# pixray/pixray

Measured on AMD Instinct MI355X. Metric: optimisation iters/sec, VQGAN 256^2 + ViT-B/32 + 64 cutouts, higher is better.
Workload: dtype fp16

## Files before the change

include/prx.h:

```cpp
#ifndef PRX_H_
#define PRX_H_
#include <stddef.h>
#include <stdint.h>

#ifdef __cplusplus
extern "C" {
#endif

#define PRX_ABI_VERSION 3

typedef void* prx_stream_t;

const char* prx_last_error(void);
int prx_abi_version(void);
int prx_device_info(int* cu_count, char* arch_name, int arch_name_len);


#define PRX_ACT_NONE 0
#define PRX_ACT_QUICKGELU 1
#define PRX_ACT_MUL_DQUICKGELU 2
#define PRX_ACT_RELU 3
#define PRX_ACT_MUL_RELUMASK 4
#define PRX_ACT_RELUMASK_POST 5
#define PRX_ACT_GELU 6
#define PRX_ACT_MUL_DGELU 7
#define PRX_A_ROWMAJOR 0
#define PRX_A_CONV3X3 1

#define PRX_PREC_BF16 0
#define PRX_PREC_F32 1
#define PRX_PREC_F16 2

typedef struct prx_gemm_ctx prx_gemm_ctx;
prx_gemm_ctx* prx_gemm_ctx_create(void);
void prx_gemm_ctx_destroy(prx_gemm_ctx* c);

typedef struct prx_gemm_args {
    const void* A;
    int a_is_f32, a_mode, lda;
    const void* B;
    int ldb;
    int M, N, K;
    int H, W, Cin, up;
    float alpha;
    const float* bias_n;
    const float* bias_m;
    const void* aux;
    int ldaux;
    const float* resid;
    int ldr;
    int act;
    float* out_f32; int ldc_f32;
    void* out_bf16; void* out_bf16_pre; int ldc_bf16;
    int f32;
    int row16;
    prx_gemm_ctx* ctx;
} prx_gemm_args;
int prx_k_gemm(const prx_gemm_args* g, void* ws, size_t ws_bytes, prx_stream_t stream);
int prx_k_gemm_gn(const prx_gemm_args* g, double* gn_stats, int gn_gs, const float* gnb_x, const double* gnb_fstats,
                  const float* gnb_gamma, const float* gnb_beta, int gnb_swish, float gnb_eps, void* ws, size_t ws_bytes,
                  prx_stream_t stream);
long long prx_gemm_fit_spec_launches(void);
long long prx_gemm_row_launches(void);

int prx_k_groupnorm_fwd(const float* x, const float* gamma, const float* beta, double* stats, void* out_bf16,
                        float* out_f32, int NB, int P, int C, int swish, float eps, prx_stream_t s);
int prx_k_groupnorm_bwd(const float* g, const float* x, const float* gamma, const float* beta, const double* fstats,
                        double* bstats, const float* add, float* dx, int NB, int P, int C, int swish, float eps,
                        prx_stream_t s);
int prx_k_layernorm_fwd(const float* x, long long ldx, const float* gamma, const float* beta, void* out_bf16,
                        float* out_f32, float* mean, float* rstd, int rows, int C, float eps, prx_stream_t s);
int prx_k_layernorm_bwd(const float* g, long long ldg, const float* x, long long ldx, const float* gamma,
                        const float* mean, const float* rstd, const float* add, long long ldadd, float* dx,
                        long long lddx, int rows, int C, prx_stream_t s);
int prx_k_transpose_bf16(const void* in, int ldin, void* out, int ldout, int R, int C, prx_stream_t s);
int prx_k_softmax_rows(const float* S, int lds_, float scale, void* P, int ldp, void* PT, int ldpt, int rows, int cols,
                       prx_stream_t s);
int prx_k_softmax_rows_bwd(const void* P, int ldp, const float* dP, int lddp, float scale, void* dS, int ldds,
                           void* dST, int lddst, int rows, int cols, prx_stream_t s);
int prx_k_upsample2x_bwd(const float* hi, float* low, int NB, int Hl, int Wl, int C, prx_stream_t s);
int prx_k_nchw_to_nhwc(const float* in, float* out_f32, void* out_bf16, int NB, int C, int HW, int Cpad,
                       prx_stream_t s);
int prx_k_nhwc_to_nchw(const float* in, int ldc, float* out, int NB, int C, int HW, prx_stream_t s);
int prx_k_image_head_fwd(const float* x, int ldc, float* img, int NB, int C, int HW, prx_stream_t s);
int prx_k_image_head_bwd(const float* x, int ldc, const float* gimg, float* dx, void* dx_bf16, int ldo, int NB, int C,
                         int HW, prx_stream_t s);
int prx_k_mha_fwd(const void* qkv, void* out, int N, int T, int C, int heads, prx_stream_t s);
int prx_k_mha_bwd(const void* qkv, const void* dout, void* dqkv, int N, int T, int C, int heads, prx_stream_t s);

int prx_k_groupnorm_fwd_op(const void* x, const float* gamma, const float* beta, double* stats, void* out16, float* out_f32,
                           int NB, int P, int C, int swish, float eps, int zero_stats, int stats_ready, int h16, int s16,
                           prx_stream_t s);
int prx_k_groupnorm_bwd_op(const void* g, const void* x, const float* gamma, const float* beta, const double* fstats,
                           double* bstats, const void* add, float* dx, void* dx16, int NB, int P, int C, int swish, float eps,
                           int zero_stats, int stats_ready, int h16, int s16, prx_stream_t s);
int prx_k_layernorm_fwd_op(const void* x, long long ldx, const float* gamma, const float* beta, void* out16, float* out_f32,
                           float* mean, float* rstd, int rows, int C, float eps, int h16, int s16, prx_stream_t s);
int prx_k_layernorm_bwd_op(const void* g, long long ldg, const void* x, long long ldx, const float* gamma, const float* mean,
                           const float* rstd, const void* add, long long ldadd, float* dx, long long lddx, void* dx16,
                           long long lddxb, int rows, int C, int h16, int add_every, int s16, prx_stream_t s);
int prx_k_mha_fwd_op(const void* qkv, void* out, int N, int T, int C, int heads, int h16, prx_stream_t s);
int prx_k_mha_bwd_op(const void* qkv, const void* dout, void* dqkv, int N, int T, int C, int heads, int h16, prx_stream_t s);
int prx_k_mha_fwd_gen_op(const void* qkv, void* out, float* lse, int N, int T, int C, int heads, int h16, prx_stream_t s);
int prx_k_mha_bwd_gen_op(const void* qkv, const void* out, const void* dout, const float* lse, void* dqkv, int N, int T, int C,
                         int heads, int h16, prx_stream_t s);
int prx_k_mha_fwd_hd_op(const void* qkv, void* out, float* lse, int N, int T, int C, int heads, int h16, int head_cols, prx_stream_t s);
int prx_k_mha_bwd_hd_op(const void* qkv, const void* out, const void* dout, const float* lse, void* dqkv, int N, int T, int C,
                        int heads, int h16, int head_cols, prx_stream_t s);
int prx_k_mha_fwd_hdim_op(const void* qkv, void* out, float* lse, int N, int T, int C, int heads, int h16, int head_cols, int head_dim,
                          prx_stream_t s);
int prx_k_mha_bwd_hdim_op(const void* qkv, const void* out, const void* dout, const float* lse, void* dqkv, int N, int T, int C,
                          int heads, int h16, int head_cols, int head_dim, prx_stream_t s);
int prx_k_layernorm_fwd_rag_op(const void* x, long long ldx, const float* gamma, const float* beta, void* out16, float* out_f32,
                               float* mean, float* rstd, int rows, int C, float eps, int h16, int s16, prx_stream_t s);
int prx_k_layernorm_bwd_rag_op(const void* g, long long ldg, const void* x, long long ldx, const float* gamma, const float* mean,
                               const float* rstd, const void* add, long long ldadd, float* dx, long long lddx, void* dx16, long long lddxb,
                               int rows, int C, int h16, int add_every, int s16, prx_stream_t s);
int prx_k_vit_pad_heads(const float* qkv_w, float* qkv_w_pad, const float* out_w, float* out_w_pad, int width, int heads, int hd, int hp,
                        prx_stream_t s);
int prx_k_mha_fwd_causal_op(const void* qkv, void* out, int N, int T, int C, int heads, int h16, prx_stream_t s);
int prx_k_softmax_rows_op(const float* S, int lds_, float scale, void* P, int ldp, void* PT, int ldpt, int rows, int cols,
                          int prec, prx_stream_t s);
int prx_k_softmax_rows_bwd_op(const void* P, int ldp, const float* dP, int lddp, float scale, void* dS, int ldds, void* dST,
                              int lddst, int rows, int cols, int prec, prx_stream_t s);
int prx_k_transpose_op(const void* in, int ldin, void* out, int ldout, int R, int C, int f32, prx_stream_t s);
int prx_k_upsample2x_bwd_op(const void* hi, float* low, void* low16, int NB, int Hl, int Wl, int C, int h16, int s16,
                            prx_stream_t s);
int prx_k_nchw_to_nhwc_op(const float* in, float* out_f32, void* out16, int NB, int C, int HW, int Cpad, int h16, prx_stream_t s);
int prx_k_image_head_bwd_op(const float* x, int ldc, const float* gimg, float* dx, void* dx16, int ldo, int NB, int C, int HW,
                            int h16, const float* gscale, prx_stream_t s);
int prx_k_image_head_bwd_im2col(const float* x, int ldc, const float* gimg, void* col, int ldk, int C, int H, int W, int h16,
                                const float* gscale, prx_stream_t s);
int prx_k_grad_scale(const float* g, size_t n, float* part, int nparts, int target_log2, float* scale2, prx_stream_t s);
int prx_k_grad_scale_multi(const float* const* gs, const size_t* ns, int count, float* part, int nparts_each, int target_log2,
                           float* scale2, prx_stream_t s);
int prx_k_scale_dev(float* x, size_t n, const float* scale, void* out16, int h16, prx_stream_t s);
int prx_k_f32_to_op16(const float* in, void* out16, size_t n, int h16, prx_stream_t s);
int prx_k_add_f32(const float* a, const float* b, float* out, size_t n, prx_stream_t s);

int prx_k_rn_pack_conv3x3(const float* w, void* Wf, void* Wd, int Cout, int Cin, int prec, prx_stream_t s);
int prx_k_stem1_fwd(const float* cut, const float* mm, const float* w, const float* b, void* out, int N, int S, int CO, int prec,
                    prx_stream_t s);
int prx_k_stem1_bwd(const void* g, const float* w, float* dY, int N, int S, int CO, const float* oscale_dev, int prec, prx_stream_t s);
int prx_k_avgpool2_fwd(const void* x, void* out, int N, int H, int W, int C, int prec, prx_stream_t s);
int prx_k_avgpool2_bwd(const float* g, const void* mask, float* dx_f32, void* dx_op, int N, int H, int W, int C, int prec,
                       prx_stream_t s);
int prx_k_relu_mask(float* g, const void* out, void* g_op, size_t n, int prec, prx_stream_t s);
int prx_k_tokens_fwd(const float* x, const float* pos, void* t, int N, int P, int C, int prec, prx_stream_t s);
int prx_k_tokens_bwd(const float* dt, float* dx, int N, int P, int C, int prec, prx_stream_t s);
int prx_k_tok0_gather(const void* t, void* out, int N, int T, int C, int prec, prx_stream_t s);
int prx_k_tok0_scatter(const void* g0, void* dt, int N, int T, int C, int prec, prx_stream_t s);
int prx_k_cnx_pack_dw(const float* w, void* pack, int C, int prec, prx_stream_t s);
int prx_k_cnx_dwconv(const void* x, const void* pack, const float* bias, const float* add, void* out_op, float* out_f32, int N, int H,
                     int W, int C, int flip, int prec, prx_stream_t s);
int prx_k_cnx_space_to_depth(const void* in, void* out, int N, int H, int W, int C, int prec, prx_stream_t s);
int prx_k_cnx_depth_to_space(const void* in, void* out, int N, int H, int W, int C, int prec, prx_stream_t s);
int prx_k_cnx_avgpool_fwd(const void* x, float* out, int N, int HW, int C, int prec, prx_stream_t s);
int prx_k_cnx_avgpool_bwd(const float* g, float* dx_f32, void* dx_op, int N, int HW, int C, int prec, prx_stream_t s);
int prx_k_cnx_layernorm_fwd(const void* x, int x_f32, const float* gamma, const float* beta, void* out_op, float* out_f32, float* mean,
                            float* rstd, int rows, int C, float eps, int group, int prec, prx_stream_t s);
int prx_k_cnx_layernorm_bwd(const float* g, const void* x, int x_f32, const float* gamma, const float* mean, const float* rstd,
                            void* dx_op, float* dx_f32, int rows, int C, int group, int prec, prx_stream_t s);
int prx_k_minmax(const float* x, size_t n, float* part, int nparts, float* mm, prx_stream_t s);
int prx_k_patchify_fwd(const float* cut, const float* mm, void* A, int prec, int N, int S, int P, int T, float m0, float m1, float m2,
                       float s0, float s1, float s2, prx_stream_t s);
int prx_k_patchify_bwd_reduce(const float* cut, const float* mm, const float* dA, double* acc, int N, int S, int P, int T, float m0,
                              float m1, float m2, float s0, float s1, float s2, prx_stream_t s);
int prx_k_patchify_bwd_apply(const float* cut, const float* mm, const float* dA, const double* acc, float* gcut, int N, int S, int P,
                             int T, float m0, float m1, float m2, float s0, float s1, float s2, prx_stream_t s);
int prx_k_preproc_bwd_reduce(const float* cut, const float* mm, const float* dY, double* acc, int N, int S, prx_stream_t s);
int prx_k_preproc_bwd_apply(const float* cut, const float* mm, const float* dY, const double* acc, float* gcut, int N, int S,
                            prx_stream_t s);
int prx_k_pool_fwd(const float* img, float* pooled, int* argmax, const unsigned char* mask, int C, int H, int W, int S, prx_stream_t s);
int prx_k_pool_bwd(const float* g, const int* argmax, const unsigned char* mask, float* gimg, int C, int H, int W, int S, prx_stream_t s);
int prx_k_rescale_fwd(const float* pooled, float* base, int C, int S, int Hb, int Wb, prx_stream_t s);
int prx_k_rescale_bwd(const float* g_base, float* g_pooled, int C, int S, int Hb, int Wb, prx_stream_t s);
int prx_k_warp_a_fwd(const float* src, int Hs, int Ws, const double* desc, float* out, int n_cut, int Ha, int Wa, prx_stream_t s);
int prx_k_warp_a_bwd(const float* g, int Hs, int Ws, const double* desc, float* uv, float* gsrc_priv, float* gsrc, int n_cut, int Ha,
                     int Wa, int form, prx_stream_t s);
int prx_k_warp_b_fwd(const float* a, int Ha, int Wa, const double* desc, const float* noise, float* out, int n_cut, int S,
                     prx_stream_t s);
int prx_k_warp_b_bwd(const float* a, int Ha, int Wa, const double* desc, const float* g, float* grgb, float* uv, float* ga, int n_cut,
                     int S, float* maps_scratch, size_t maps_scratch_bytes, int form, prx_stream_t s);
int prx_cutout_bwd_separable(int on);
int prx_k_vgg_pack(const float* w, void* Wf, void* Wd, int Cout, int Cin, int CiP, int prec, prx_stream_t s);
int prx_k_vgg_input(const float* x, void* out, int HW, int prec, prx_stream_t s);
int prx_k_vgg_input_grad(const float* d, float* gx, int HW, const float* unscale, prx_stream_t s);
int prx_k_vgg_maxpool(const void* x, void* out, void* arg, int H, int W, int C, int prec, prx_stream_t s);
int prx_k_vgg_combine(const float* above, const void* arg, const float* gcap, const void* act, void* gpre, int H, int W, int C,
                      const float* gscale, int prec, prx_stream_t s);
int prx_k_pack_transpose_op(const float* in, void* out, int R, int C, int prec, prx_stream_t s);
int prx_k_vit_add_cls_pos(float* x, const float* cls, const float* pos, int N, int T, int W, prx_stream_t s);
int prx_k_vit_embed_tokens(const float* x, const float* cls, const float* pos, void* out, int out16, int N, int T, int W,
                           prx_stream_t s);
int prx_k_vit_gelu_f32(const float* t, float* io, size_t n, int bwd, prx_stream_t s);
int prx_k_vit_scale_f32(float* x, size_t n, float scale, int blocks, prx_stream_t s);
int prx_k_text_embed(const int* tokens, const float* emb, const float* pos, float* x, int* eot, int n, int ctx, int W, int vocab,
                     prx_stream_t s);
int prx_k_gather_rows(const float* x, const int* eot, float* out, int n, int ctx, int W, prx_stream_t s);
int prx_k_l2norm_fwd(const float* e, float* out, int n, int D, prx_stream_t s);
int prx_k_l2norm_bwd(const float* e, const float* g, float* de, int n, int D, prx_stream_t s);
int prx_k_vqgan_pack_conv3x3(const float* w, void* Wf, void* Wd, int Cout, int Cin, int CoP, int prec, prx_stream_t s);
int prx_k_vqgan_enc_pack_conv3x3(const float* w, void* Wf, int Cout, int Cin, int CiP, prx_stream_t s);
int prx_k_colminmax(const float* w, float* mn, float* mx, int rows, int D, prx_stream_t s);


typedef struct prx_vqgan prx_vqgan;
// ... 329 lines not shown
```

pixray_amd/csrc/api_core.hip:

```cpp
#include "common.h"
#include "gemm.h"
#include "../../include/prx.h"
#include <stdarg.h>
#include <stdio.h>
#include <string.h>
#include <stdlib.h>

static thread_local char g_err[1024] = "";

void prx_set_error(const char* fmt, ...) {
    va_list ap;
    va_start(ap, fmt);
    vsnprintf(g_err, sizeof(g_err), fmt, ap);
    va_end(ap);
}

int prx_xcd_local() {
    static const int v = getenv("PRX_XCD_LOCAL") ? atoi(getenv("PRX_XCD_LOCAL")) : 1;
    return v;
}

int prx_grad_target_log2() {
    static const int v = [] {
        const char* e = getenv("PRX_GRAD_TARGET_LOG2");
        int k = e ? atoi(e) : 4;
        return k < -8 ? -8 : (k > 14 ? 14 : k);
    }();
    return v;
}

extern "C" {

const char* prx_last_error(void) { return g_err; }

int prx_abi_version(void) { return PRX_ABI_VERSION; }

int prx_device_info(int* cu_count, char* arch_name, int arch_name_len) {
    int dev = 0;
    PRX_CHECK_HIP(hipGetDevice(&dev));
    hipDeviceProp_t p;
    PRX_CHECK_HIP(hipGetDeviceProperties(&p, dev));
    if (cu_count) *cu_count = p.multiProcessorCount;
    if (arch_name && arch_name_len > 0) {
        strncpy(arch_name, p.gcnArchName, arch_name_len - 1);
        arch_name[arch_name_len - 1] = 0;
    }
    return 0;
}

static int desc_of(const prx_gemm_args* g, GemmDesc& d) {
    PRX_REQUIRE(g != nullptr, "prx_k_gemm: null args");
    PRX_REQUIRE(prec_valid(g->f32), "prx_k_gemm: unknown operand precision %d", g->f32);
    d.f32 = prec_is_f32(g->f32); d.h16 = prec_is_h16(g->f32);
    d.A = g->A; d.a_is_f32 = g->a_is_f32; d.a_mode = g->a_mode; d.lda = g->lda;
    d.B = g->B; d.ldb = g->ldb;
    d.M = g->M; d.N = g->N; d.K = g->K;
    d.H = g->H; d.W = g->W; d.Cin = g->Cin; d.up = g->up;
    d.alpha = g->alpha;
    d.bias_n = g->bias_n; d.bias_m = g->bias_m;
    d.aux = g->aux; d.ldaux = g->ldaux;
    d.resid = g->resid; d.ldr = g->ldr;
    d.act = g->act;
    d.out_f32 = g->out_f32; d.ldc_f32 = g->ldc_f32;
    d.out_bf16 = g->out_bf16; d.out_bf16_pre = g->out_bf16_pre;
    d.ldc_bf16 = g->ldc_bf16;
    d.row16 = (short)(g->row16 & 3);
    return 0;
}
int prx_k_gemm(const prx_gemm_args* g, void* ws, size_t ws_bytes, prx_stream_t stream_) {
    GemmDesc d;
    int r = desc_of(g, d);
    if (r) return r;
    return prx_gemm_launch(d, (float*)ws, ws_bytes, (hipStream_t)stream_, (GemmCtx*)g->ctx);
}
int prx_k_gemm_gn(const prx_gemm_args* g, double* gn_stats, int gn_gs, const float* gnb_x, const double* gnb_fstats,
                  const float* gnb_gamma, const float* gnb_beta, int gnb_swish, float gnb_eps, void* ws, size_t ws_bytes,
                  prx_stream_t stream_) {
    GemmDesc d;
    int r = desc_of(g, d);
    if (r) return r;
    PRX_REQUIRE(gn_stats != nullptr, "prx_k_gemm_gn: null gn_stats");
    d.gn_stats = gn_stats; d.gn_gs = gn_gs;
    d.gnb_x = gnb_x; d.gnb_fstats = gnb_fstats; d.gnb_gamma = gnb_gamma; d.gnb_beta = gnb_beta; d.gnb_swish = gnb_swish; d.gnb_eps = gnb_eps;
    return prx_gemm_launch(d, (float*)ws, ws_bytes, (hipStream_t)stream_, (GemmCtx*)g->ctx);
}

prx_gemm_ctx* prx_gemm_ctx_create(void) { return (prx_gemm_ctx*)new GemmCtx(); }
void prx_gemm_ctx_destroy(prx_gemm_ctx* c) { delete (GemmCtx*)c; }
void prx_profile_gemm_enable(prx_gemm_ctx* c, int on) { prx_gemm_ctx_profile_enable((GemmCtx*)c, on); }
void prx_gemm_tile_override(prx_gemm_ctx* c, int bm, int bn, int splits) { prx_gemm_ctx_force_tile((GemmCtx*)c, bm, bn, splits); }
int prx_gemm_plan(prx_gemm_ctx* c, const prx_gemm_args* g, size_t ws_bytes, int n_cu, int* out) {
    GemmDesc d;
    int r = desc_of(g, d);
    if (r) return r;
    GemmPlan p;
    r = prx_gemm_plan_impl(d, (const GemmCtx*)c, n_cu, ws_bytes, true, &p);
    if (r) return r;
    const GemmLaunchPlan& l0 = p.launch[0], l1 = p.n_launch == 2 ? p.launch[1] : GemmLaunchPlan{};
    const int o[9] = {l0.family, l0.bm, l0.bn, l0.splits, p.rows_8p, p.n_launch == 2 ? (int)l1.family : -1, l1.bm, l1.bn, p.n_launch == 2 ? l1.splits : 0};
    memcpy(out, o, sizeof o);
    return 0;
}
int prx_gemm_plan_rows_8phase(prx_gemm_ctx* c, int M, int N, int K) {
    if (M <= 0 || N <= 0 || K <= 0) return 0;
    prx_gemm_args g = {};
    g.a_mode = PRX_A_ROWMAJOR; g.lda = g.ldb = K; g.M = M; g.N = N; g.K = K; g.alpha = 1.f;
    int out[9];
    return prx_gemm_plan(c, &g, 0, c ? ((GemmCtx*)c)->n_cu : 0, out) == 0 ? out[4] : 0;
}
void prx_gemm_tile_rule(prx_gemm_ctx* c, int M, int N, int K, int mode, int bm, int bn, int splits) {
    prx_gemm_ctx_tile_rule((GemmCtx*)c, M, N, K, mode, bm, bn, splits);
}
int prx_profile_gemm_collect(prx_gemm_ctx* c, double* total_ms, double* total_flop, long long* launches) {
    return prx_gemm_ctx_profile_collect((GemmCtx*)c, total_ms, total_flop, launches);
}

}
```

pixray_amd/csrc/api_kernels.hip:

```cpp
#include "common.h"
#include "norms.h"
#include "elementwise.h"
#include "attention.h"
#include "resnet.h"
#include "convnext.h"
#include "cutouts.h"
#include "vgg.h"
#include "vit.h"
#include "clip_text.h"
#include "prompt_vq.h"
#include "vqgan.h"
#include "vqgan_enc.h"
#include "fft_drawer.h"
#include "../../include/prx.h"

#define S_(x) ((hipStream_t)(x))
#define B_(x) ((bf16_t*)(x))
#define CB_(x) ((const bf16_t*)(x))

extern "C" {

int prx_k_groupnorm_fwd(const float* x, const float* gamma, const float* beta, double* stats, void* out_bf16,
                        float* out_f32, int NB, int P, int C, int swish, float eps, prx_stream_t s) {
    return prx_groupnorm_fwd(x, gamma, beta, stats, B_(out_bf16), out_f32, NB, P, C, swish, eps, S_(s));
// ... 101 lines not shown
                             stats_ready, h16, s16);
}
int prx_k_layernorm_fwd_op(const void* x, long long ldx, const float* gamma, const float* beta, void* out16, float* out_f32,
                           float* mean, float* rstd, int rows, int C, float eps, int h16, int s16, prx_stream_t s) {
    return prx_layernorm_fwd(x, ldx, gamma, beta, B_(out16), out_f32, mean, rstd, rows, C, eps, S_(s), h16, s16);
}
int prx_k_layernorm_bwd_op(const void* g, long long ldg, const void* x, long long ldx, const float* gamma, const float* mean,
                           const float* rstd, const void* add, long long ldadd, float* dx, long long lddx, void* dx16,
                           long long lddxb, int rows, int C, int h16, int add_every, int s16, prx_stream_t s) {
    return prx_layernorm_bwd(g, ldg, x, ldx, gamma, mean, rstd, add, ldadd, dx, lddx, B_(dx16), lddxb, rows, C, S_(s), h16,
                             add_every, s16);
}
int prx_k_mha_fwd_op(const void* qkv, void* out, int N, int T, int C, int heads, int h16, prx_stream_t s) {
    return prx_mha_fwd(CB_(qkv), B_(out), N, T, C, heads, S_(s), h16);
}
int prx_k_mha_bwd_op(const void* qkv, const void* dout, void* dqkv, int N, int T, int C, int heads, int h16, prx_stream_t s) {
    return prx_mha_bwd(CB_(qkv), CB_(dout), B_(dqkv), N, T, C, heads, S_(s), h16);
}
int prx_k_mha_fwd_gen_op(const void* qkv, void* out, float* lse, int N, int T, int C, int heads, int h16, prx_stream_t s) {
    return prx_mha_fwd_gen(CB_(qkv), B_(out), lse, N, T, C, heads, S_(s), h16);
}
int prx_k_mha_bwd_gen_op(const void* qkv, const void* out, const void* dout, const float* lse, void* dqkv, int N, int T, int C,
                         int heads, int h16, prx_stream_t s) {
    return prx_mha_bwd_gen(CB_(qkv), CB_(out), CB_(dout), lse, B_(dqkv), N, T, C, heads, S_(s), h16);
}
int prx_k_mha_fwd_hd_op(const void* qkv, void* out, float* lse, int N, int T, int C, int heads, int h16, int head_cols, prx_stream_t s) {
    PRX_REQUIRE(head_cols == 64 || head_cols == 96, "mha_fwd_hd: %d columns per head (64 | 96)", head_cols);
    if (head_cols == 64) return prx_mha_fwd_gen(CB_(qkv), B_(out), lse, N, T, C, heads, S_(s), h16);
    return prx_mha_fwd_hd96(CB_(qkv), B_(out), lse, N, T, C, heads, 1.f / sqrtf(80.f), S_(s), h16);
}
int prx_k_mha_bwd_hd_op(const void* qkv, const void* out, const void* dout, const float* lse, void* dqkv, int N, int T, int C,
                        int heads, int h16, int head_cols, prx_stream_t s) {
    PRX_REQUIRE(head_cols == 64 || head_cols == 96, "mha_bwd_hd: %d columns per head (64 | 96)", head_cols);
    if (head_cols == 64) return prx_mha_bwd_gen(CB_(qkv), CB_(out), CB_(dout), lse, B_(dqkv), N, T, C, heads, S_(s), h16);
    return prx_mha_bwd_hd96(CB_(qkv), CB_(out), CB_(dout), lse, B_(dqkv), N, T, C, heads, 1.f / sqrtf(80.f), S_(s), h16);
}
int prx_k_mha_fwd_hdim_op(const void* qkv, void* out, float* lse, int N, int T, int C, int heads, int h16, int head_cols, int head_dim,
                          prx_stream_t s) {
    PRX_REQUIRE(head_dim >= 64 && prx_vit_head_cols(head_dim) == head_cols, "mha_fwd_hdim: head dim %d at %d columns per head (64 at 64, 80 | 88 at 96, 104 at 128)",
                head_dim, head_cols);
    const float scale = 1.f / sqrtf((float)head_dim);
    if (head_cols == 64) return prx_mha_fwd_gen(CB_(qkv), B_(out), lse, N, T, C, heads, S_(s), h16);
    if (head_cols == 96) return prx_mha_fwd_hd96(CB_(qkv), B_(out), lse, N, T, C, heads, scale, S_(s), h16);
    return prx_mha_fwd_hd128(CB_(qkv), B_(out), lse, N, T, C, heads, scale, S_(s), h16);
}
int prx_k_mha_bwd_hdim_op(const void* qkv, const void* out, const void* dout, const float* lse, void* dqkv, int N, int T, int C,
                          int heads, int h16, int head_cols, int head_dim, prx_stream_t s) {
    PRX_REQUIRE(head_dim >= 64 && prx_vit_head_cols(head_dim) == head_cols, "mha_bwd_hdim: head dim %d at %d columns per head (64 at 64, 80 | 88 at 96, 104 at 128)",
                head_dim, head_cols);
    const float scale = 1.f / sqrtf((float)head_dim);
    if (head_cols == 64) return prx_mha_bwd_gen(CB_(qkv), CB_(out), CB_(dout), lse, B_(dqkv), N, T, C, heads, S_(s), h16);
    if (head_cols == 96) return prx_mha_bwd_hd96(CB_(qkv), CB_(out), CB_(dout), lse, B_(dqkv), N, T, C, heads, scale, S_(s), h16);
    return prx_mha_bwd_hd128(CB_(qkv), CB_(out), CB_(dout), lse, B_(dqkv), N, T, C, heads, scale, S_(s), h16);
}
int prx_k_layernorm_fwd_rag_op(const void* x, long long ldx, const float* gamma, const float* beta, void* out16, float* out_f32,
                               float* mean, float* rstd, int rows, int C, float eps, int h16, int s16, prx_stream_t s) {
    return prx_layernorm_fwd(x, ldx, gamma, beta, B_(out16), out_f32, mean, rstd, rows, C, eps, S_(s), h16, s16, 1);
}
int prx_k_layernorm_bwd_rag_op(const void* g, long long ldg, const void* x, long long ldx, const float* gamma, const float* mean,
                               const float* rstd, const void* add, long long ldadd, float* dx, long long lddx, void* dx16, long long lddxb,
                               int rows, int C, int h16, int add_every, int s16, prx_stream_t s) {
    return prx_layernorm_bwd(g, ldg, x, ldx, gamma, mean, rstd, add, ldadd, dx, lddx, B_(dx16), lddxb, rows, C, S_(s), h16,
                             add_every, s16, 1);
}
int prx_k_vit_pad_heads(const float* qkv_w, float* qkv_w_pad, const float* out_w, float* out_w_pad, int width, int heads, int hd, int hp,
                        prx_stream_t s) {
    PRX_REQUIRE(qkv_w && qkv_w_pad && out_w && out_w_pad && width == heads * hd, "vit_pad_heads: null argument or width != heads * head dim");
    int r = prx_vit_pad_head_rows(qkv_w, qkv_w_pad, heads, hd, hp, width, S_(s));
    return r ? r : prx_vit_pad_head_cols(out_w, out_w_pad, width, heads, hd, hp, S_(s));
}
int prx_k_mha_fwd_causal_op(const void* qkv, void* out, int N, int T, int C, int heads, int h16, prx_stream_t s) {
    return prx_mha_fwd_causal(CB_(qkv), B_(out), N, T, C, heads, S_(s), h16);
}
int prx_k_softmax_rows_op(const float* S, int lds_, float scale, void* P, int ldp, void* PT, int ldpt, int rows, int cols,
                          int prec, prx_stream_t s) {
    PRX_REQUIRE(prec_valid(prec), "softmax_rows: unknown precision %d", prec);
    return prx_softmax_rows(S, lds_, scale, P, ldp, PT, ldpt, rows, cols, prec, S_(s));
}
int prx_k_softmax_rows_bwd_op(const void* P, int ldp, const float* dP, int lddp, float scale, void* dS, int ldds, void* dST,
                              int lddst, int rows, int cols, int prec, prx_stream_t s) {
    PRX_REQUIRE(prec_valid(prec), "softmax_rows_bwd: unknown precision %d", prec);
    return prx_softmax_rows_bwd(P, ldp, dP, lddp, scale, dS, ldds, dST, lddst, rows, cols, prec, S_(s));
}
int prx_k_transpose_op(const void* in, int ldin, void* out, int ldout, int R, int C, int f32, prx_stream_t s) {
    return prx_transpose_op(in, ldin, out, ldout, R, C, f32, S_(s));
}
int prx_k_upsample2x_bwd_op(const void* hi, float* low, void* low16, int NB, int Hl, int Wl, int C, int h16, int s16,
                            prx_stream_t s) {
    return prx_upsample2x_bwd(hi, low, B_(low16), NB, Hl, Wl, C, S_(s), h16, s16);
}
int prx_k_nchw_to_nhwc_op(const float* in, float* out_f32, void* out16, int NB, int C, int HW, int Cpad, int h16, prx_stream_t s) {
    return prx_nchw_to_nhwc(in, out_f32, B_(out16), NB, C, HW, Cpad, S_(s), h16);
}
int prx_k_image_head_bwd_op(const float* x, int ldc, const float* gimg, float* dx, void* dx16, int ldo, int NB, int C, int HW,
                            int h16, const float* gscale, prx_stream_t s) {
    return prx_image_head_bwd(x, ldc, gimg, dx, B_(dx16), ldo, NB, C, HW, S_(s), h16, gscale);
}
int prx_k_image_head_bwd_im2col(const float* x, int ldc, const float* gimg, void* col, int ldk, int C, int H, int W, int h16,
                                const float* gscale, prx_stream_t s) {
    return prx_image_head_bwd_im2col(x, ldc, gimg, B_(col), ldk, C, H, W, S_(s), h16, gscale);
}
int prx_k_grad_scale(const float* g, size_t n, float* part, int nparts, int target_log2, float* scale2, prx_stream_t s) {
    return prx_grad_scale(g, n, part, nparts, target_log2, scale2, S_(s));
}
int prx_k_grad_scale_multi(const float* const* gs, const size_t* ns, int count, float* part, int nparts_each, int target_log2,
                           float* scale2, prx_stream_t s) {
    return prx_grad_scale_multi(gs, ns, count, part, nparts_each, target_log2, scale2, S_(s));
}
int prx_k_scale_dev(float* x, size_t n, const float* scale, void* out16, int h16, prx_stream_t s) {
    return prx_scale_dev(x, n, scale, S_(s), B_(out16), h16);
}
int prx_k_f32_to_op16(const float* in, void* out16, size_t n, int h16, prx_stream_t s) {
    return prx_f32_to_bf16(in, B_(out16), n, S_(s), h16);
}
int prx_k_add_f32(const float* a, const float* b, float* out, size_t n, prx_stream_t s) {
    return prx_add_f32(a, b, out, n, S_(s));
}

int prx_k_rn_pack_conv3x3(const float* w, void* Wf, void* Wd, int Cout, int Cin, int prec, prx_stream_t s) {
    return prx_rn_pack_conv3x3(w, Wf, Wd, Cout, Cin, prec, S_(s));
}
int prx_k_stem1_fwd(const float* cut, const float* mm, const float* w, const float* b, void* out, int N, int S, int CO, int prec, prx_stream_t s) {
    return prx_stem1_fwd(cut, mm, w, b, out, N, S, CO, prec, S_(s));
}
int prx_k_stem1_bwd(const void* g, const float* w, float* dY, int N, int S, int CO, const float* oscale_dev, int prec, prx_stream_t s) {
    return prx_stem1_bwd(g, w, dY, N, S, CO, oscale_dev, prec, S_(s));
}
int prx_k_avgpool2_fwd(const void* x, void* out, int N, int H, int W, int C, int prec, prx_stream_t s) {
    return prx_avgpool2_fwd(x, out, N, H, W, C, prec, S_(s));
}
int prx_k_avgpool2_bwd(const float* g, const void* mask, float* dx_f32, void* dx_op, int N, int H, int W, int C, int prec, prx_stream_t s) {
    return prx_avgpool2_bwd(g, mask, dx_f32, dx_op, N, H, W, C, prec, S_(s));
}
int prx_k_relu_mask(float* g, const void* out, void* g_op, size_t n, int prec, prx_stream_t s) {
    return prx_relu_mask(g, out, g_op, n, prec, S_(s));
}
int prx_k_tokens_fwd(const float* x, const float* pos, void* t, int N, int P, int C, int prec, prx_stream_t s) {
    return prx_tokens_fwd(x, pos, t, N, P, C, prec, S_(s));
}
int prx_k_tokens_bwd(const float* dt, float* dx, int N, int P, int C, int prec, prx_stream_t s) {
    return prx_tokens_bwd(dt, dx, N, P, C, prec, S_(s));
}
int prx_k_tok0_gather(const void* t, void* out, int N, int T, int C, int prec, prx_stream_t s) {
    return prx_tok0_gather(t, out, N, T, C, prec, S_(s));
}
int prx_k_tok0_scatter(const void* g0, void* dt, int N, int T, int C, int prec, prx_stream_t s) {
    return prx_tok0_scatter(g0, dt, N, T, C, prec, S_(s));
}
int prx_k_minmax(const float* x, size_t n, float* part, int nparts, float* mm, prx_stream_t s) {
    return prx_minmax(x, n, part, nparts, mm, S_(s));
}
int prx_k_patchify_fwd(const float* cut, const float* mm, void* A, int prec, int N, int S, int P, int T, float m0, float m1, float m2, float s0, float s1, float s2, prx_stream_t s) {
    return prx_patchify_fwd(cut, mm, A, prec, N, S, P, T, S_(s), PatchNorm{{m0, m1, m2}, {s0, s1, s2}});
}
int prx_k_patchify_bwd_reduce(const float* cut, const float* mm, const float* dA, double* acc, int N, int S, int P, int T, float m0, float m1, float m2, float s0, float s1, float s2, prx_stream_t s) {
    return prx_patchify_bwd_reduce(cut, mm, dA, acc, N, S, P, T, S_(s), PatchNorm{{m0, m1, m2}, {s0, s1, s2}});
}
int prx_k_patchify_bwd_apply(const float* cut, const float* mm, const float* dA, const double* acc, float* gcut, int N, int S, int P, int T, float m0, float m1, float m2, float s0, float s1, float s2, prx_stream_t s) {
    return prx_patchify_bwd_apply(cut, mm, dA, acc, gcut, N, S, P, T, S_(s), PatchNorm{{m0, m1, m2}, {s0, s1, s2}});
}
int prx_k_preproc_bwd_reduce(const float* cut, const float* mm, const float* dY, double* acc, int N, int S, prx_stream_t s) {
    return prx_preproc_bwd_reduce(cut, mm, dY, acc, N, S, S_(s));
}
int prx_k_preproc_bwd_apply(const float* cut, const float* mm, const float* dY, const double* acc, float* gcut, int N, int S, prx_stream_t s) {
    return prx_preproc_bwd_apply(cut, mm, dY, acc, gcut, N, S, S_(s));
}
// ... 117 lines not shown
```

pixray_amd/csrc/elementwise.h:

```cpp
#pragma once
#include "common.h"
int prx_transpose_op(const void* in, int ldin, void* out, int ldout, int R, int C, int f32, hipStream_t s);
int prx_softmax_rows(const float* S, int lds_, float scale, void* P, int ldp, void* PT, int ldpt, int rows,
                     int cols, int prec, hipStream_t s);
int prx_softmax_rows_bwd(const void* P, int ldp, const float* dP, int lddp, float scale, void* dS, int ldds,
                         void* dST, int lddst, int rows, int cols, int prec, hipStream_t s);
int prx_upsample2x_bwd(const void* hi, float* low, bf16_t* low_bf16, int NB, int Hl, int Wl, int C, hipStream_t s, int h16 = 0, int s16 = 0);
int prx_nchw_to_nhwc(const float* in, float* out_f32, bf16_t* out_bf16, int NB, int C, int HW, int Cpad, hipStream_t s, int h16 = 0);
int prx_nhwc_to_nchw(const float* in, int ldc, float* out, int NB, int C, int HW, hipStream_t s);
int prx_image_head_fwd(const float* x, int ldc, float* img, int NB, int C, int HW, hipStream_t s);
int prx_image_head_bwd(const float* x, int ldc, const float* gimg, float* dx, bf16_t* dx_bf16, int ldo, int NB, int C,
                       int HW, hipStream_t s, int h16 = 0, const float* gscale = nullptr);
int prx_image_head_bwd_im2col(const float* x, int ldc, const float* gimg, bf16_t* col, int ldk, int C, int H, int W, hipStream_t s, int h16 = 0,
                              const float* gscale = nullptr);
int prx_grad_scale(const float* g, size_t n, float* part, int nparts, int target_log2, float* scale2, hipStream_t s);
int prx_adam_clamp(float* z, float* m, float* v, const float* g, const float* zmin, const float* zmax, int hw,
                   size_t n, float lr, float b1, float b2, float eps, int step, hipStream_t s);
int prx_adam_clamp_dev(float* z, float* m, float* v, const float* g, const float* zmin, const float* zmax, int hw,
                       size_t n, const float* hyper, float b1, float b2, float eps, hipStream_t s);
int prx_f32_to_bf16(const float* in, bf16_t* out, size_t n, hipStream_t s, int h16 = 0);
int prx_grad_scale_multi(const float* const* gs, const size_t* ns, int count, float* part, int nparts_each, int target_log2,
                         float* scale2, hipStream_t s);
int prx_add_f32(const float* a, const float* b, float* out, size_t n, hipStream_t s);
int prx_scale_dev(float* x, size_t n, const float* scale, hipStream_t s, bf16_t* out16 = nullptr, int h16 = 0);
```

pixray_amd/csrc/elementwise.hip:

```cpp
#include "elementwise.h"
#include <algorithm>

namespace {

inline int ew_grid(size_t total, int per = 256) { return (int)std::min<size_t>((total + per - 1) / per, 8192); }

template <typename T>
__global__ __launch_bounds__(256) void transpose_op_kernel(const T* __restrict__ in, int ldin,
                                                           T* __restrict__ out, int ldout, int R, int C) {
    __shared__ T tile[32][33];
    const int tx = threadIdx.x & 31, ty = threadIdx.x >> 5;
    const int r0 = blockIdx.y * 32, c0 = blockIdx.x * 32;
#pragma unroll
    for (int i = 0; i < 4; ++i) {
        int r = r0 + ty + 8 * i, c = c0 + tx;
        tile[ty + 8 * i][tx] = (r < R && c < C) ? in[(size_t)r * ldin + c] : (T)0.f;
    }
    __syncthreads();
#pragma unroll
    for (int i = 0; i < 4; ++i) {
        int c = c0 + ty + 8 * i, r = r0 + tx;
        if (c < C && r < R) out[(size_t)c * ldout + r] = tile[tx][ty + 8 * i];
    }
}

template <typename T>
__global__ __launch_bounds__(256) void softmax_rows_kernel(const float* __restrict__ S, int lds_, float scale,
                                                           T* __restrict__ P, int ldp, T* __restrict__ PT,
                                                           int ldpt, int rows, int cols) {
    const int lane = threadIdx.x & 63;
    const int row = blockIdx.x * 4 + (threadIdx.x >> 6);
    if (row >= rows) return;
    const float* s = S + (size_t)row * lds_;
    float mx = -INFINITY;
    for (int c = lane; c < cols; c += 64) mx = fmaxf(mx, s[c] * scale);
    mx = wave_max(mx);
    float sum = 0.f;
    for (int c = lane; c < cols; c += 64) sum += __expf(s[c] * scale - mx);
    sum = wave_sum(sum);
    const float inv = 1.f / sum;
    for (int c = lane; c < cols; c += 64) {
        T p = op_cvt<T>(__expf(s[c] * scale - mx) * inv);
        P[(size_t)row * ldp + c] = p;
        if (PT) PT[(size_t)c * ldpt + row] = p;
    }
}

template <typename T>
__global__ __launch_bounds__(256) void softmax_rows_bwd_kernel(const T* __restrict__ P, int ldp,
                                                               const float* __restrict__ dP, int lddp, float scale,
                                                               T* __restrict__ dS, int ldds,
                                                               T* __restrict__ dST, int lddst, int rows, int cols) {
    const int lane = threadIdx.x & 63;
    const int row = blockIdx.x * 4 + (threadIdx.x >> 6);
    if (row >= rows) return;
    float dot = 0.f;
    for (int c = lane; c < cols; c += 64)
        dot += (float)P[(size_t)row * ldp + c] * dP[(size_t)row * lddp + c];
    dot = wave_sum(dot);
    for (int c = lane; c < cols; c += 64) {
        float p = (float)P[(size_t)row * ldp + c];
        T v = op_cvt<T>(scale * p * (dP[(size_t)row * lddp + c] - dot));
        dS[(size_t)row * ldds + c] = v;
        if (dST) dST[(size_t)c * lddst + row] = v;
    }
}

template <bool S16>
__global__ __launch_bounds__(256) void upsample2x_bwd_kernel(const void* __restrict__ hi, float* __restrict__ low,
                                                             bf16_t* __restrict__ low_bf16, int NB, int Hl, int Wl,
                                                             int C, int h16) {
    const int C4 = C >> 2;
    const size_t total = (size_t)NB * Hl * Wl * C4;
    const int Wh = Wl * 2;
    for (size_t idx = (size_t)blockIdx.x * blockDim.x + threadIdx.x; idx < total;
         idx += (size_t)gridDim.x * blockDim.x) {
        int cq = (int)(idx % C4);
        size_t pix = idx / C4;
        int x = (int)(pix % Wl);
        size_t t = pix / Wl;
        int y = (int)(t % Hl);
        int b = (int)(t / Hl);
        size_t p00 = (((size_t)b * Hl * 2 + 2 * y) * Wh + 2 * x) * C4 + cq;
        float4 a = stream_ld4<S16>(hi, p00, h16), bb = stream_ld4<S16>(hi, p00 + C4, h16), c = stream_ld4<S16>(hi, p00 + (size_t)Wh * C4, h16),
               d = stream_ld4<S16>(hi, p00 + (size_t)Wh * C4 + C4, h16);
        float4 o = make_float4((a.x + bb.x) + (c.x + d.x), (a.y + bb.y) + (c.y + d.y), (a.z + bb.z) + (c.z + d.z),
                               (a.w + bb.w) + (c.w + d.w));
        if (low) reinterpret_cast<float4*>(low)[idx] = o;
        if (low_bf16) {
            reinterpret_cast<bf16x4*>(low_bf16)[idx] = to_op16x4(o.x, o.y, o.z, o.w, h16);
        }
    }
}

__global__ __launch_bounds__(256) void nchw_to_nhwc_kernel(const float* __restrict__ in, float* __restrict__ out_f32,
                                                           bf16_t* __restrict__ out_bf16, int NB, int C, int HW,
                                                           int Cpad, int h16) {
    const size_t total = (size_t)NB * HW * Cpad;
    for (size_t idx = (size_t)blockIdx.x * blockDim.x + threadIdx.x; idx < total;
         idx += (size_t)gridDim.x * blockDim.x) {
        int c = (int)(idx % Cpad);
        size_t t = idx / Cpad;
        int p = (int)(t % HW);
        int b = (int)(t / HW);
        float v = c < C ? in[((size_t)b * C + c) * HW + p] : 0.f;
        if (out_f32) out_f32[idx] = v;
        if (out_bf16) out_bf16[idx] = to_op16(v, h16);
    }
}

__global__ __launch_bounds__(256) void nhwc_to_nchw_kernel(const float* __restrict__ in, int ldc,
                                                           float* __restrict__ out, int NB, int C, int HW) {
    const size_t total = (size_t)NB * C * HW;
    for (size_t idx = (size_t)blockIdx.x * blockDim.x + threadIdx.x; idx < total;
         idx += (size_t)gridDim.x * blockDim.x) {
        int p = (int)(idx % HW);
        size_t t = idx / HW;
        int c = (int)(t % C);
        int b = (int)(t / C);
        out[idx] = in[((size_t)b * HW + p) * ldc + c];
    }
}

__global__ __launch_bounds__(256) void image_head_fwd_kernel(const float* __restrict__ x, int ldc,
                                                             float* __restrict__ img, int NB, int C, int HW) {
    const size_t total = (size_t)NB * C * HW;
    for (size_t idx = (size_t)blockIdx.x * blockDim.x + threadIdx.x; idx < total;
         idx += (size_t)gridDim.x * blockDim.x) {
        int p = (int)(idx % HW);
        size_t t = idx / HW;
        int c = (int)(t % C);
        int b = (int)(t / C);
        float v = (x[((size_t)b * HW + p) * ldc + c] + 1.f) * 0.5f;
        img[idx] = fminf(fmaxf(v, 0.f), 1.f);
    }
}

__global__ __launch_bounds__(256) void image_head_bwd_kernel(const float* __restrict__ x, int ldc,
                                                             const float* __restrict__ gimg, float* __restrict__ dx,
                                                             bf16_t* __restrict__ dx_bf16, int ldo, int NB, int C,
                                                             int HW, int h16, const float* __restrict__ gscale_dev) {
    const float gscale = gscale_dev ? *gscale_dev : 1.f;
    const size_t total = (size_t)NB * HW * ldo;
    for (size_t idx = (size_t)blockIdx.x * blockDim.x + threadIdx.x; idx < total;
         idx += (size_t)gridDim.x * blockDim.x) {
        int c = (int)(idx % ldo);
        size_t t = idx / ldo;
        int p = (int)(t % HW);
// ... 64 lines not shown
}

__global__ __launch_bounds__(256) void f32_to_bf16_kernel(const float* __restrict__ in, bf16_t* __restrict__ out,
                                                          size_t n, int h16) {
    for (size_t i = (size_t)blockIdx.x * blockDim.x + threadIdx.x; i < n; i += (size_t)gridDim.x * blockDim.x)
        out[i] = to_op16(in[i], h16);
}

__global__ __launch_bounds__(256) void amax_partial_kernel(const float* __restrict__ g, size_t n, float* __restrict__ part) {
    float m = 0.f;
    for (size_t i = (size_t)blockIdx.x * blockDim.x + threadIdx.x; i < n; i += (size_t)gridDim.x * blockDim.x) {
        const float a = fabsf(g[i]);
        m = fmaxf(m, a == a ? a : INFINITY);
    }
    m = wave_max(m);
    __shared__ float s[4];
    if ((threadIdx.x & 63) == 0) s[threadIdx.x >> 6] = m;
    __syncthreads();
    if (threadIdx.x == 0) part[blockIdx.x] = fmaxf(fmaxf(s[0], s[1]), fmaxf(s[2], s[3]));
}
__global__ __launch_bounds__(256) void grad_scale_final_kernel(const float* __restrict__ part, int nparts, int target_log2,
                                                               float* __restrict__ scale2) {
    float m = 0.f;
    for (int i = threadIdx.x; i < nparts; i += blockDim.x) m = fmaxf(m, part[i]);
    m = wave_max(m);
    __shared__ float s[4];
    if ((threadIdx.x & 63) == 0) s[threadIdx.x >> 6] = m;
    __syncthreads();
    if (threadIdx.x == 0) {
        m = fmaxf(fmaxf(s[0], s[1]), fmaxf(s[2], s[3]));
        float S = 1.f;
        if (m > 0.f && m < INFINITY) {
            int e;
            (void)frexpf(m, &e);
            int k = target_log2 - e;
            k = k < -40 ? -40 : (k > 60 ? 60 : k);
            S = ldexpf(1.f, k);
        }
        scale2[0] = S;
        scale2[1] = 1.f / S;
    }
}

__global__ __launch_bounds__(256) void scale_dev_kernel(float* __restrict__ x, size_t n, const float* __restrict__ scale, bf16_t* __restrict__ out16, int h16) {
    const float sc = *scale;
    for (size_t i = (size_t)blockIdx.x * blockDim.x + threadIdx.x; i < n; i += (size_t)gridDim.x * blockDim.x) {
        const float v = x[i] * sc;
        x[i] = v;
        if (out16) out16[i] = to_op16(v, h16);
    }
}

__global__ __launch_bounds__(256) void add_f32_kernel(const float* __restrict__ a, const float* __restrict__ b,
                                                      float* __restrict__ out, size_t n) {
    for (size_t i = (size_t)blockIdx.x * blockDim.x + threadIdx.x; i < n; i += (size_t)gridDim.x * blockDim.x)
        out[i] = a[i] + b[i];
}

}

int prx_transpose_op(const void* in, int ldin, void* out, int ldout, int R, int C, int f32, hipStream_t s) {
    dim3 grid(ceil_div(C, 32), ceil_div(R, 32));
    if (f32) hipLaunchKernelGGL(transpose_op_kernel<float>, grid, dim3(256), 0, s, (const float*)in, ldin, (float*)out, ldout, R, C);
    else     hipLaunchKernelGGL(transpose_op_kernel<bf16_t>, grid, dim3(256), 0, s, (const bf16_t*)in, ldin, (bf16_t*)out, ldout, R, C);
    PRX_LAUNCH_CHECK();
    return 0;
}
int prx_softmax_rows(const float* S, int lds_, float scale, void* P, int ldp, void* PT, int ldpt, int rows,
                     int cols, int prec, hipStream_t s) {
    PRX_OP_DISPATCH(prec_is_f32(prec), prec_is_h16(prec), T,
                    hipLaunchKernelGGL(softmax_rows_kernel<T>, dim3(ceil_div(rows, 4)), dim3(256), 0, s, S, lds_, scale, (T*)P, ldp,
                                       (T*)PT, ldpt, rows, cols));
    PRX_LAUNCH_CHECK();
    return 0;
}
int prx_softmax_rows_bwd(const void* P, int ldp, const float* dP, int lddp, float scale, void* dS, int ldds,
                         void* dST, int lddst, int rows, int cols, int prec, hipStream_t s) {
    PRX_OP_DISPATCH(prec_is_f32(prec), prec_is_h16(prec), T,
                    hipLaunchKernelGGL(softmax_rows_bwd_kernel<T>, dim3(ceil_div(rows, 4)), dim3(256), 0, s, (const T*)P, ldp, dP, lddp,
                                       scale, (T*)dS, ldds, (T*)dST, lddst, rows, cols));
    PRX_LAUNCH_CHECK();
    return 0;
}
int prx_upsample2x_bwd(const void* hi, float* low, bf16_t* low_bf16, int NB, int Hl, int Wl, int C, hipStream_t s, int h16, int s16) {
    PRX_REQUIRE(C % 4 == 0 && (low || low_bf16), "upsample2x_bwd: C %% 4 != 0, or no output");
    if (s16) hipLaunchKernelGGL(upsample2x_bwd_kernel<true>, dim3(ew_grid((size_t)NB * Hl * Wl * C / 4)), dim3(256), 0, s, hi, low, low_bf16,
                                NB, Hl, Wl, C, h16);
    else hipLaunchKernelGGL(upsample2x_bwd_kernel<false>, dim3(ew_grid((size_t)NB * Hl * Wl * C / 4)), dim3(256), 0, s, hi, low, low_bf16,
                            NB, Hl, Wl, C, h16);
    PRX_LAUNCH_CHECK();
    return 0;
}
int prx_nchw_to_nhwc(const float* in, float* out_f32, bf16_t* out_bf16, int NB, int C, int HW, int Cpad,
                     hipStream_t s, int h16) {
    hipLaunchKernelGGL(nchw_to_nhwc_kernel, dim3(ew_grid((size_t)NB * HW * Cpad)), dim3(256), 0, s, in, out_f32,
                       out_bf16, NB, C, HW, Cpad, h16);
    PRX_LAUNCH_CHECK();
    return 0;
}
int prx_nhwc_to_nchw(const float* in, int ldc, float* out, int NB, int C, int HW, hipStream_t s) {
    hipLaunchKernelGGL(nhwc_to_nchw_kernel, dim3(ew_grid((size_t)NB * HW * C)), dim3(256), 0, s, in, ldc, out, NB, C,
                       HW);
    PRX_LAUNCH_CHECK();
    return 0;
}
int prx_image_head_fwd(const float* x, int ldc, float* img, int NB, int C, int HW, hipStream_t s) {
    hipLaunchKernelGGL(image_head_fwd_kernel, dim3(ew_grid((size_t)NB * HW * C)), dim3(256), 0, s, x, ldc, img, NB, C,
                       HW);
    PRX_LAUNCH_CHECK();
    return 0;
}
int prx_grad_scale(const float* g, size_t n, float* part, int nparts, int target_log2, float* scale2, hipStream_t s) {
    PRX_REQUIRE(nparts >= 1 && nparts <= 1024, "grad_scale: 1..1024 partials");
    const int blocks = (int)std::min<size_t>((n + 1023) / 1024 + 1, (size_t)nparts);
    hipLaunchKernelGGL(amax_partial_kernel, dim3(blocks), dim3(256), 0, s, g, n, part);
    PRX_LAUNCH_CHECK();
    hipLaunchKernelGGL(grad_scale_final_kernel, dim3(1), dim3(256), 0, s, part, blocks, target_log2, scale2);
    PRX_LAUNCH_CHECK();
    return 0;
}
int prx_grad_scale_multi(const float* const* gs, const size_t* ns, int count, float* part, int nparts_each, int target_log2,
                         float* scale2, hipStream_t s) {
    PRX_REQUIRE(count >= 1 && nparts_each >= 1 && (long long)count * nparts_each <= 4096, "grad_scale_multi: bad partial layout");
    int used = 0;
    for (int i = 0; i < count; ++i) {
        if (!gs[i] || ns[i] == 0) continue;
        const int blocks = (int)std::min<size_t>((ns[i] + 1023) / 1024 + 1, (size_t)nparts_each);
        hipLaunchKernelGGL(amax_partial_kernel, dim3(blocks), dim3(256), 0, s, gs[i], ns[i], part + used);
        PRX_LAUNCH_CHECK();
        used += blocks;
    }
    PRX_REQUIRE(used > 0, "grad_scale_multi: no gradient tensor");
    hipLaunchKernelGGL(grad_scale_final_kernel, dim3(1), dim3(256), 0, s, part, used, target_log2, scale2);
    PRX_LAUNCH_CHECK();
    return 0;
}
int prx_scale_dev(float* x, size_t n, const float* scale, hipStream_t s, bf16_t* out16, int h16) {
    hipLaunchKernelGGL(scale_dev_kernel, dim3(ew_grid(n)), dim3(256), 0, s, x, n, scale, out16, h16);
    PRX_LAUNCH_CHECK();
    return 0;
}
int prx_image_head_bwd(const float* x, int ldc, const float* gimg, float* dx, bf16_t* dx_bf16, int ldo, int NB, int C,
                       int HW, hipStream_t s, int h16, const float* gscale) {
    hipLaunchKernelGGL(image_head_bwd_kernel, dim3(ew_grid((size_t)NB * HW * ldo)), dim3(256), 0, s, x, ldc, gimg, dx,
                       dx_bf16, ldo, NB, C, HW, h16, gscale);
    PRX_LAUNCH_CHECK();
    return 0;
}
int prx_image_head_bwd_im2col(const float* x, int ldc, const float* gimg, bf16_t* col, int ldk, int C, int H, int W, hipStream_t s, int h16,
                              const float* gscale) {
    PRX_REQUIRE(C <= 8 && ldk % 8 == 0 && ldk >= 72, "image_head_bwd_im2col: at most 8 channels, row pitch a multiple of 8 >= 72");
    hipLaunchKernelGGL(image_head_bwd_im2col_kernel, dim3(ew_grid((size_t)H * W * (ldk / 8))), dim3(256), 0, s, x, ldc, gimg, col, ldk, C, H, W,
                       h16, gscale);
    PRX_LAUNCH_CHECK();
    return 0;
}
int prx_adam_clamp(float* z, float* m, float* v, const float* g, const float* zmin, const float* zmax, int hw,
                   size_t n, float lr, float b1, float b2, float eps, int step, hipStream_t s) {
    PRX_REQUIRE(step >= 1, "adam: step must be >= 1");
    const double bc1 = 1.0 - pow((double)b1, step);
    const double bc2 = 1.0 - pow((double)b2, step);
    hipLaunchKernelGGL(adam_clamp_kernel, dim3(ew_grid(n)), dim3(256), 0, s, z, m, v, g, zmin, zmax, hw, n, lr, b1, b2,
                       eps, (float)bc1, (float)sqrt(bc2), (const float*)nullptr);
    PRX_LAUNCH_CHECK();
    return 0;
}
// ... 19 lines not shown
```

pixray_amd/csrc/gemm.h:

```cpp
#pragma once
#include "common.h"
#include <vector>
#include <mutex>

enum { PRX_ACT_NONE = 0, PRX_ACT_QUICKGELU = 1, PRX_ACT_MUL_DQUICKGELU = 2,
       PRX_ACT_RELU = 3,
       PRX_ACT_MUL_RELUMASK = 4,
       PRX_ACT_RELUMASK_POST = 5,
       PRX_ACT_GELU = 6,
       PRX_ACT_MUL_DGELU = 7 };
inline __host__ __device__ bool prx_act_needs_aux(int act) {
    return act == PRX_ACT_MUL_DQUICKGELU || act == PRX_ACT_MUL_RELUMASK || act == PRX_ACT_RELUMASK_POST || act == PRX_ACT_MUL_DGELU;
}
inline __host__ __device__ bool prx_act_saves_pre(int act) { return act == PRX_ACT_QUICKGELU || act == PRX_ACT_GELU; }
enum { PRX_A_ROWMAJOR = 0, PRX_A_CONV3X3 = 1 };

struct GemmDesc {
    int f32 = 0;
    int h16 = 0;
    const void* A = nullptr;
    int a_is_f32 = 0;
    int a_mode = PRX_A_ROWMAJOR;
    int lda = 0;
    const void* B = nullptr;
    int ldb = 0;
    int M = 0, N = 0, K = 0;
    int H = 0, W = 0, Cin = 0, up = 0;
    float alpha = 1.f;
    const float* alpha_dev = nullptr;
    const float* bias_n = nullptr;
    const float* bias_m = nullptr;
    const void* aux = nullptr; int ldaux = 0;
    const float* resid = nullptr; int ldr = 0;
    int act = PRX_ACT_NONE;
    float* out_f32 = nullptr; int ldc_f32 = 0;
    void* out_bf16 = nullptr;
    void* out_bf16_pre = nullptr;
    int ldc_bf16 = 0;
    double* gn_stats = nullptr;
    int gn_gs = 0;
    const float* gnb_x = nullptr;
    const double* gnb_fstats = nullptr;
    const float* gnb_gamma = nullptr;
    const float* gnb_beta = nullptr;
    short gnb_swish = 0;
    short row16 = 0;
    float gnb_eps = 1e-6f;
};

struct GemmTileRule { int M, N, K, mode, bm, bn, splits; };
struct GemmProfRec { hipEvent_t a, b; double flop; int M, N, K, mode, bm, bn, splits; };
struct GemmCtx {
    int use_glds = 1;
    int force_bm = 0, force_bn = 0, force_splits = 0, force_stages = 0;
    int xcd_swizzle = 2;
    int conv_c64 = 1;
    int wide_tile = 128;
    int tile8p = 128;
    int fit_flags = 1;
    int n_cu = 0;
    int n_cu_dev = -1;
    int force_fit = 0;
    int dbg_only = -2, dbg_count = 0;
    int fit_conv = 1;
    int fit = 1;
    int rowk = 1;
    int rowk_min = 24 << 20;
    std::vector<GemmTileRule> rules;
    bool prof_on = false;
    std::vector<GemmProfRec> prof;
    std::mutex mu;
    GemmCtx();
};
enum GemmFamily { GEMM_TILED_V1 = 0, GEMM_TILED_GLDS = 1, GEMM_TILED_F32 = 2, GEMM_FIT = 3, GEMM_8PHASE = 4, GEMM_ROW = 5, GEMM_ROWCONV = 6 };
struct GemmLaunchPlan {
    GemmFamily family = GEMM_TILED_GLDS;
    int bm = 0, bn = 0;
    int splits = 1, kt_per_split = 0;
    int stages = 2;
    bool c64 = false;
    int vec_epi = 0, xcd_swizzle = 0, fit_flags = 0;
    int row_nt = 0, row_ksm = 0;
};
struct GemmPlan {
    GemmLaunchPlan launch[2];
    int n_launch = 0;
    int rows_8p = 0;
    bool stats_pass = false;
    int dbg_used = 0;
};
int prx_gemm_plan_impl(const GemmDesc& d, const GemmCtx* c, int n_cu, size_t ws_bytes, bool ws_al16, GemmPlan* p);

void prx_gemm_ctx_force_tile(GemmCtx* c, int bm, int bn, int splits);
void prx_gemm_ctx_tile_rule(GemmCtx* c, int M, int N, int K, int mode, int bm, int bn, int splits);
void prx_gemm_ctx_profile_enable(GemmCtx* c, int on);
int prx_gemm_ctx_profile_collect(GemmCtx* c, double* total_ms, double* total_flop, long long* launches);

int prx_gemm_launch(const GemmDesc& d, float* ws, size_t ws_bytes, hipStream_t stream, GemmCtx* ctx = nullptr);
```

pixray_amd/csrc/gemm.hip:

```cpp
#include "gemm_epi.h"
#include "norms.h"
#include <vector>
#include <mutex>
#include <stdlib.h>
#include <type_traits>

namespace {

constexpr int BK = 64;
constexpr int LDS_LD = BK + 8;

using namespace prx_gemm_dev;

template <typename T16>
__device__ __forceinline__ f32x16 mfma16(const bf16x8& a, const bf16x8& b, const f32x16& c) {
    if constexpr (std::is_same<T16, half_t>::value)
        return __builtin_amdgcn_mfma_f32_32x32x16_f16(__builtin_bit_cast(f16x8, a), __builtin_bit_cast(f16x8, b), c, 0, 0, 0);
    else
        return __builtin_amdgcn_mfma_f32_32x32x16_bf16(a, b, c, 0, 0, 0);
}
template <typename T16, typename TA>
__device__ __forceinline__ bf16x8 load8(const TA* p) {
    if constexpr (std::is_same<TA, float>::value) {
        f32x4 a = *reinterpret_cast<const f32x4*>(p);
        f32x4 b = *reinterpret_cast<const f32x4*>(p + 4);
        typedef __attribute__((ext_vector_type(8))) T16 t16x8;
        t16x8 r;
        r[0] = op_cvt<T16>(a[0]); r[1] = op_cvt<T16>(a[1]); r[2] = op_cvt<T16>(a[2]); r[3] = op_cvt<T16>(a[3]);
        r[4] = op_cvt<T16>(b[0]); r[5] = op_cvt<T16>(b[1]); r[6] = op_cvt<T16>(b[2]); r[7] = op_cvt<T16>(b[3]);
        return __builtin_bit_cast(bf16x8, r);
    } else {
        return *reinterpret_cast<const bf16x8*>(p);
    }
}

template <int BM, int BN, typename TA, int AMODE, typename T16 = bf16_t>
__global__ __launch_bounds__(256) void gemm_kernel(const GemmArgs p) {
    constexpr int A_CH = BM * 8 / 256;
    constexpr int B_CH = BN * 8 / 256;
    constexpr int MT = BM / 64;
    constexpr int NT = BN / 64;

    __shared__ __attribute__((aligned(16))) bf16_t As[BM * LDS_LD];
    __shared__ __attribute__((aligned(16))) bf16_t Bs[BN * LDS_LD];

    const GemmDesc& d = p.d;
    const int tid = threadIdx.x;
    const int lane = tid & 63;
    const int wave = tid >> 6;
    const int wm = wave >> 1, wn = wave & 1;

    const int bid = blockIdx.x;
    const int tm = bid / p.tiles_n;
    const int tn = bid - tm * p.tiles_n;
    const int split = blockIdx.y;
    const int kt0 = split * p.kt_per_split;
    const int kt1 = min(p.kt_total, kt0 + p.kt_per_split);

    const TA* __restrict__ Ap = reinterpret_cast<const TA*>(d.A);
    const bf16_t* __restrict__ Bp = reinterpret_cast<const bf16_t*>(d.B);

    int a_row[A_CH];
    long long a_base[A_CH];
    int a_y[A_CH], a_x[A_CH], a_b[A_CH];
    bool a_ok[A_CH];
    const int kc = tid & 7;
#pragma unroll
    for (int i = 0; i < A_CH; ++i) {
        int row = (tid >> 3) + 32 * i;
        a_row[i] = row;
        int gm = tm * BM + row;
        a_ok[i] = gm < d.M;
        if (AMODE == PRX_A_ROWMAJOR) {
            a_base[i] = (long long)gm * d.lda;
            a_y[i] = a_x[i] = a_b[i] = 0;
        } else {
            int hw = d.H * d.W;
            int b = gm / hw;
            int rem = gm - b * hw;
            int y = rem / d.W;
            a_b[i] = b; a_y[i] = y; a_x[i] = rem - y * d.W;
            a_base[i] = 0;
        }
    }
    int b_row[B_CH];
    long long b_base[B_CH];
// ... 204 lines not shown
                const long long pix = ((long long)a_b[i] * Hs + yy) * Ws + xx;
                a_reg[i] = ok ? *reinterpret_cast<const f32x4*>(Ap + pix * d.lda + c) : zero4;
            }
        }
#pragma unroll
        for (int i = 0; i < B_CH; ++i)
            b_reg[i] = (b_ok[i] && k_ok) ? *reinterpret_cast<const f32x4*>(Bp + b_base[i] + k) : zero4;
    };
    auto store_tiles = [&]() __attribute__((always_inline)) {
#pragma unroll
        for (int i = 0; i < A_CH; ++i)
            *reinterpret_cast<f32x4*>(&As[a_row[i] * LDS_LDF + kc * 4]) = a_reg[i];
#pragma unroll
        for (int i = 0; i < B_CH; ++i)
            *reinterpret_cast<f32x4*>(&Bs[b_row[i] * LDS_LDF + kc * 4]) = b_reg[i];
    };

    f32x16 acc[MT][NT];
#pragma unroll
    for (int i = 0; i < MT; ++i)
#pragma unroll
        for (int j = 0; j < NT; ++j)
#pragma unroll
            for (int r = 0; r < 16; ++r) acc[i][j][r] = 0.f;

    if (kt0 < kt1) {
        load_tiles(kt0);
        store_tiles();
    }
    __syncthreads();

    const int frag_row = lane & 31;
    const int frag_k = 4 * (lane >> 5);
    for (int kt = kt0; kt < kt1; ++kt) {
        const bool more = (kt + 1) < kt1;
        if (more) load_tiles(kt + 1);
#pragma unroll
        for (int ks = 0; ks < BKF / 8; ++ks) {
            f32x4 af[MT], bfr[NT];
#pragma unroll
            for (int i = 0; i < MT; ++i)
                af[i] = *reinterpret_cast<const f32x4*>(&As[(wm * (BM / 2) + i * 32 + frag_row) * LDS_LDF + ks * 8 + frag_k]);
#pragma unroll
            for (int j = 0; j < NT; ++j)
                bfr[j] = *reinterpret_cast<const f32x4*>(&Bs[(wn * (BN / 2) + j * 32 + frag_row) * LDS_LDF + ks * 8 + frag_k]);
#pragma unroll
            for (int e = 0; e < 4; ++e)
#pragma unroll
                for (int i = 0; i < MT; ++i)
#pragma unroll
                    for (int j = 0; j < NT; ++j)
                        acc[i][j] = __builtin_amdgcn_mfma_f32_32x32x2f32(af[i][e], bfr[j][e], acc[i][j], 0, 0, 0);
        }
        __syncthreads();
        if (more) {
            store_tiles();
            __syncthreads();
        }
    }

    const int row0 = tm * BM + wm * (BM / 2) + 4 * (lane >> 5);
    const int col0 = tn * BN + wn * (BN / 2) + (lane & 31);
#pragma unroll
    for (int i = 0; i < MT; ++i)
#pragma unroll
        for (int j = 0; j < NT; ++j) {
            const int col = col0 + j * 32;
            if (col >= d.N) continue;
#pragma unroll
            for (int r = 0; r < 16; ++r) {
                const int row = row0 + i * 32 + (r & 3) + 8 * (r >> 2);
                if (row >= d.M) continue;
                if (p.splits > 1)
                    p.ws[((size_t)split * d.M + row) * d.N + col] = acc[i][j][r];
                else
                    epilogue_store<float>(d, row, col, acc[i][j][r]);
            }
        }
}

typedef const __attribute__((address_space(1))) void* gptr_t;
typedef __attribute__((address_space(3))) void* lptr_t;

template <int BM, int BN, int AMODE, int STAGES, bool C64 = false, int NWM = 2, typename T16 = bf16_t>
__global__ __launch_bounds__(NWM * 128) void gemm_glds_kernel(const GemmArgs p, const bf16_t* __restrict__ zero_page) {
    constexpr int NW = NWM * 2;
    constexpr int A_IN = BM / (8 * NW);
    constexpr int B_IN = BN / (8 * NW);
    constexpr int MT = BM / (32 * NWM);
    constexpr int NT = BN / 64;
    static_assert(A_IN >= 1 && B_IN >= 1 && MT >= 1 && NT >= 1, "tile too small for the wave grid");
    constexpr int TILE = (BM + BN) * BK;

    __shared__ __attribute__((aligned(16))) bf16_t lds[STAGES * TILE];

    const GemmDesc& d = p.d;
    const int tid = threadIdx.x;
    const int lane = tid & 63;
    const int wave = __builtin_amdgcn_readfirstlane(tid >> 6);
    const int wm = wave >> 1, wn = wave & 1;

    int bid = blockIdx.x;
    if (p.xcd_swizzle) {
        const int nwg = gridDim.x, xcd = bid & 7, local = bid >> 3;
        const int q = nwg >> 3, r = nwg & 7;
        bid = (xcd < r ? xcd * (q + 1) : r * (q + 1) + (xcd - r) * q) + local;
    }
    const int tm = bid / p.tiles_n;
    const int tn = bid - tm * p.tiles_n;
    const int split = blockIdx.y;
    const int kt0 = split * p.kt_per_split;
    const int kt1 = min(p.kt_total, kt0 + p.kt_per_split);

    const bf16_t* __restrict__ Ap = reinterpret_cast<const bf16_t*>(d.A);
    const bf16_t* __restrict__ Bp = reinterpret_cast<const bf16_t*>(d.B);

    const int lrow = lane >> 3, cpos = lane & 7;
    long long a_base[A_IN];
    int a_sw[A_IN], a_y[A_IN], a_x[A_IN], a_b[A_IN];
    bool a_ok[A_IN];
#pragma unroll
    for (int i = 0; i < A_IN; ++i) {
        const int row = (wave * A_IN + i) * 8 + lrow;
        a_sw[i] = cpos ^ ((row >> 1) & 7);
        const int gm = tm * BM + row;
        a_ok[i] = gm < d.M;
        if (AMODE == PRX_A_ROWMAJOR) {
            a_base[i] = (long long)gm * d.lda;
            a_y[i] = a_x[i] = a_b[i] = 0;
        } else {
            const int hw = d.H * d.W;
            const int b = gm / hw;
            const int rem = gm - b * hw;
            const int y = rem / d.W;
            a_b[i] = b; a_y[i] = y; a_x[i] = rem - y * d.W;
            a_base[i] = 0;
        }
    }
    int c_r1[C64 ? A_IN : 1], c_rd0[C64 ? A_IN : 1], c_rd2[C64 ? A_IN : 1];
    int c_c1[C64 ? A_IN : 1], c_cd0[C64 ? A_IN : 1], c_cd2[C64 ? A_IN : 1], c_ok[C64 ? A_IN : 1];
    if constexpr (C64) {
        const int Hs = d.up == 1 ? (d.H >> 1) : (d.up == 2 ? 2 * d.H : d.H);
        const int Ws = d.up == 1 ? (d.W >> 1) : (d.up == 2 ? 2 * d.W : d.W);
#pragma unroll
        for (int i = 0; i < A_IN; ++i) {
            int okm = 0, ro[3], co[3];
#pragma unroll
            for (int t = 0; t < 3; ++t) {
                if (d.up == 2) {
                    const int yy = 2 * a_y[i] + t, xx = 2 * a_x[i] + t;
                    if (a_ok[i] && yy < Hs) okm |= 1 << t;
                    if (xx < Ws) okm |= 8 << t;
                    ro[t] = (a_b[i] * Hs + yy) * Ws;
                    co[t] = xx;
                } else {
                    const int yy = a_y[i] + t - 1, xx = a_x[i] + t - 1;
                    if (a_ok[i] && yy >= 0 && yy < d.H) okm |= 1 << t;
                    if (xx >= 0 && xx < d.W) okm |= 8 << t;
                    ro[t] = (a_b[i] * Hs + (d.up ? (yy >> 1) : yy)) * Ws;
                    co[t] = d.up ? (xx >> 1) : xx;
                }
            }
            c_ok[i] = okm;
            c_r1[i] = ro[1]; c_rd0[i] = ro[0] - ro[1]; c_rd2[i] = ro[2] - ro[1];
            c_c1[i] = co[1]; c_cd0[i] = co[0] - co[1]; c_cd2[i] = co[2] - co[1];
        }
    }
    int c_tap = 0, c_c0 = 0;
    if constexpr (C64) { c_tap = (kt0 * BK) / d.Cin; c_c0 = kt0 * BK - c_tap * d.Cin; }

    long long b_base[B_IN];
    int b_sw[B_IN];
    bool b_ok[B_IN];
#pragma unroll
    for (int i = 0; i < B_IN; ++i) {
        const int row = (wave * B_IN + i) * 8 + lrow;
        b_sw[i] = cpos ^ ((row >> 1) & 7);
        const int gn = tn * BN + row;
        b_ok[i] = gn < d.N;
// ... 219 lines not shown
        const size_t iters = (total4 + stride - 1) / stride;
        for (size_t it = 0; it < iters; ++it) {
            const size_t i4 = base + it * stride;
            const bool live = i4 < total4;
            float s0 = 0.f, s1 = 0.f;
            int col = 0;
            if (live) {
                float4 v = make_float4(0.f, 0.f, 0.f, 0.f);
                const float4* part = reinterpret_cast<const float4*>(p.ws) + i4;
                const size_t pstride = total >> 2;
                int s = 0;
                for (; s + 4 <= p.splits; s += 4) {
                    const float4 w0 = part[(size_t)s * pstride], w1 = part[(size_t)(s + 1) * pstride];
                    const float4 w2 = part[(size_t)(s + 2) * pstride], w3 = part[(size_t)(s + 3) * pstride];
                    v.x += w0.x; v.y += w0.y; v.z += w0.z; v.w += w0.w;
                    v.x += w1.x; v.y += w1.y; v.z += w1.z; v.w += w1.w;
                    v.x += w2.x; v.y += w2.y; v.z += w2.z; v.w += w2.w;
                    v.x += w3.x; v.y += w3.y; v.z += w3.z; v.w += w3.w;
                }
                for (; s < p.splits; ++s) {
                    const float4 w = part[(size_t)s * pstride];
                    v.x += w.x; v.y += w.y; v.z += w.z; v.w += w.w;
                }
                const size_t idx = i4 << 2;
                const int row = (int)(idx / d.N);
                col = (int)(idx - (size_t)row * d.N);
                const float4 o = epilogue_store4<TOp>(d, row, col, v);
                if (do_stats && d.gnb_x) gnb_accum<TOp>(d, gnb_load(d, col), row, col, o, s0, s1);
                else {
                    s0 = (o.x + o.y) + (o.z + o.w);
                    s1 = (o.x * o.x + o.y * o.y) + (o.z * o.z + o.w * o.w);
                }
            }
            if (do_stats) {
                for (int o = 1; o < run && o < 64; o <<= 1) { s0 += __shfl_xor(s0, o, 64); s1 += __shfl_xor(s1, o, 64); }
                if (live && (threadIdx.x & (run - 1)) == 0) {
                    const int g = col / d.gn_gs;
                    atomicAdd(&gacc[g * 2], (double)s0);
                    atomicAdd(&gacc[g * 2 + 1], (double)s1);
                }
            }
        }
        if (do_stats) {
            __syncthreads();
            if (threadIdx.x < 64 && gacc[threadIdx.x] != 0.0) atomicAdd(&d.gn_stats[threadIdx.x], gacc[threadIdx.x]);
        }
        return;
    }
    for (size_t idx = (size_t)blockIdx.x * blockDim.x + threadIdx.x; idx < total;
         idx += (size_t)gridDim.x * blockDim.x) {
        float v = 0.f;
        for (int s = 0; s < p.splits; ++s) v += p.ws[(size_t)s * total + idx];
        int row = (int)(idx / d.N);
        int col = (int)(idx - (size_t)row * d.N);
        epilogue_store<TOp>(d, row, col, v);
    }
}

template <int BM, int BN, typename T16>
void launch_cfg_t(const GemmArgs& a, dim3 grid, hipStream_t s) {
    const GemmDesc& d = a.d;
    if (d.a_mode == PRX_A_ROWMAJOR) {
        if (d.a_is_f32) hipLaunchKernelGGL((gemm_kernel<BM, BN, float, PRX_A_ROWMAJOR, T16>), grid, dim3(256), 0, s, a);
        else            hipLaunchKernelGGL((gemm_kernel<BM, BN, bf16_t, PRX_A_ROWMAJOR, T16>), grid, dim3(256), 0, s, a);
    } else {
        if (d.a_is_f32) hipLaunchKernelGGL((gemm_kernel<BM, BN, float, PRX_A_CONV3X3, T16>), grid, dim3(256), 0, s, a);
        else            hipLaunchKernelGGL((gemm_kernel<BM, BN, bf16_t, PRX_A_CONV3X3, T16>), grid, dim3(256), 0, s, a);
    }
}
template <int BM, int BN>
void launch_cfg(const GemmArgs& a, dim3 grid, hipStream_t s) {
    if (a.d.h16) launch_cfg_t<BM, BN, half_t>(a, grid, s);
    else         launch_cfg_t<BM, BN, bf16_t>(a, grid, s);
}
template <int BM, int BN>
void launch_f32(const GemmArgs& a, dim3 grid, hipStream_t s) {
    if (a.d.a_mode == PRX_A_ROWMAJOR) hipLaunchKernelGGL((gemm_f32_kernel<BM, BN, PRX_A_ROWMAJOR>), grid, dim3(256), 0, s, a);
    else                              hipLaunchKernelGGL((gemm_f32_kernel<BM, BN, PRX_A_CONV3X3>), grid, dim3(256), 0, s, a);
}

template <int BM, int BN, int STAGES, typename T16>
void launch_glds_t(const GemmArgs& a, dim3 grid, hipStream_t s, const bf16_t* zero_page, bool c64) {
    if (a.d.a_mode == PRX_A_ROWMAJOR)
        hipLaunchKernelGGL((gemm_glds_kernel<BM, BN, PRX_A_ROWMAJOR, STAGES, false, 2, T16>), grid, dim3(256), 0, s, a, zero_page);
    else if (c64)
        hipLaunchKernelGGL((gemm_glds_kernel<BM, BN, PRX_A_CONV3X3, STAGES, true, 2, T16>), grid, dim3(256), 0, s, a, zero_page);
    else
        hipLaunchKernelGGL((gemm_glds_kernel<BM, BN, PRX_A_CONV3X3, STAGES, false, 2, T16>), grid, dim3(256), 0, s, a, zero_page);
}
template <int BM, int BN, int STAGES>
void launch_glds_s(const GemmArgs& a, dim3 grid, hipStream_t s, const bf16_t* zero_page, bool c64) {
    if (a.d.h16) launch_glds_t<BM, BN, STAGES, half_t>(a, grid, s, zero_page, c64);
    else         launch_glds_t<BM, BN, STAGES, bf16_t>(a, grid, s, zero_page, c64);
}
template <int BM, int BN>
void launch_glds(const GemmArgs& a, dim3 grid, hipStream_t s, const bf16_t* zero_page, int stages, bool c64) {
    if (stages >= 4 && (BM + BN) * BK * 2 * 4 <= 160 * 1024) launch_glds_s<BM, BN, 4>(a, grid, s, zero_page, c64);
    else if (stages >= 3) launch_glds_s<BM, BN, 3>(a, grid, s, zero_page, c64);
    else launch_glds_s<BM, BN, 2>(a, grid, s, zero_page, c64);
}

std::mutex g_zero_mu;
bf16_t* g_zero_page[16] = {nullptr};

const bf16_t* zero_page_for_current_device() {
    int dev = 0;
    if (hipGetDevice(&dev) != hipSuccess || dev < 0 || dev >= 16) return nullptr;
    std::lock_guard<std::mutex> lk(g_zero_mu);
    if (!g_zero_page[dev]) {
        void* p = nullptr;
        if (hipMalloc(&p, 256) != hipSuccess) return nullptr;
        if (hipMemset(p, 0, 256) != hipSuccess) return nullptr;
        g_zero_page[dev] = (bf16_t*)p;
    }
    return g_zero_page[dev];
}

}
const bf16_t* prx_gemm_zero_page() { return zero_page_for_current_device(); }
namespace {

int env_int(const char* name, int dflt) { const char* v = getenv(name); return v ? atoi(v) : dflt; }

}

GemmCtx::GemmCtx() {
    force_stages = env_int("PRX_GEMM_STAGES", 0);
    xcd_swizzle = env_int("PRX_XCD_SWIZZLE", 2);
    conv_c64 = env_int("PRX_CONV_C64", 1);
    wide_tile = env_int("PRX_WIDE_TILE", 128);
    tile8p = env_int("PRX_GEMM_8P", 128);
    fit = env_int("PRX_GEMM_FIT", 1);
    fit_flags = env_int("PRX_FIT_FLAGS", 1);
    fit_conv = env_int("PRX_FIT_CONV", 1);
    use_glds = env_int("PRX_GEMM_V1", 0) ? 0 : 1;
    rowk = env_int("PRX_GEMM_ROWK", 1);
    rowk_min = env_int("PRX_GEMM_ROWK_MIN", 24 << 20);
}

void prx_gemm_ctx_tile_rule(GemmCtx* c, int M, int N, int K, int mode, int bm, int bn, int splits) {
    if (!c) return;
    if (M <= 0) { c->rules.clear(); return; }
    for (size_t i = 0; i < c->rules.size(); ++i)
        if (c->rules[i].M == M && c->rules[i].N == N && c->rules[i].K == K && c->rules[i].mode == mode) { c->rules.erase(c->rules.begin() + i); break; }
    const bool known = (bm == 64 && bn == 64) || (bm == 128 && (bn == 64 || bn == 128)) || (bm == 256 && (bn == 128 || bn == 256));
    if (bm > 0 && known) c->rules.push_back({M, N, K, mode, bm, bn, splits});
}

void prx_gemm_ctx_force_tile(GemmCtx* c, int bm, int bn, int splits) {
    if (!c) return;
    if (bm == -1) { c->xcd_swizzle = splits; return; }
    if (bm == -2) { c->force_stages = splits; return; }
    if (bm == -3) { c->use_glds = splits; return; }
    if (bm == -5) { c->conv_c64 = splits; return; }
    if (bm == -6) { c->tile8p = splits; return; }
    if (bm == -7) { c->fit = splits; return; }
    if (bm == -8) { c->fit_flags = splits; return; }
    if (bm == -12) { c->force_fit = splits; return; }
    if (bm == -9) { c->fit_conv = splits; return; }
    if (bm == -14) { c->rowk_min = splits > 0 ? splits : (24 << 20); return; }
    if (bm == -13) { c->dbg_only = splits; c->dbg_count = 0; return; }
    if (bm < 0) return;
    c->force_bm = bm; c->force_bn = bn; c->force_splits = splits;
}

void prx_gemm_ctx_profile_enable(GemmCtx* c, int on) {
    if (!c) return;
    std::lock_guard<std::mutex> lk(c->mu);
    c->prof_on = on != 0;
}

int prx_gemm_ctx_profile_collect(GemmCtx* c, double* total_ms, double* total_flop, long long* launches) {
    double ms = 0, fl = 0;
    long long n = 0;
    if (c) {
        std::lock_guard<std::mutex> lk(c->mu);
        FILE* dump = getenv("PRX_GEMM_PROFILE_DUMP") ? fopen(getenv("PRX_GEMM_PROFILE_DUMP"), "a") : nullptr;
        for (auto& r : c->prof) {
            float t = 0;
            if (hipEventSynchronize(r.b) != hipSuccess || hipEventElapsedTime(&t, r.a, r.b) != hipSuccess) {
                if (dump) fclose(dump);
                return -1;
// ... 115 lines not shown
        }
    }
    int bm = 128, bn = 128;
    bool want_fit = false;
    if (row) { bm = 16; bn = p->family == GEMM_ROWCONV ? 80 : 16 * p->row_nt; }
    else if (p->family == GEMM_8PHASE) { bm = bn = 256; }
    else if (rule) { bm = rule->bm; bn = rule->bn; want_fit = prx_gemmfit_tile(bm, bn, nullptr) && !fourwave_tile(bm, bn); }
    else if (cx.force_bm) { bm = cx.force_bm; bn = cx.force_bn; want_fit = prx_gemmfit_tile(bm, bn, nullptr) && (cx.force_fit || !fourwave_tile(bm, bn)); }
    else if (fbm) { bm = fbm; bn = fbn; want_fit = true; }
    else fourwave_heuristic(d, cx, n_cu, &bm, &bn);
    const bool fit_takes = want_fit && prx_gemmfit_eligible(d, bm, bn);
    const bool fit = fit_takes && p->vec_epi;
    if ((fit_takes && !fit) || (want_fit && !fit_takes && !fourwave_tile(bm, bn)) || (bm == 256 && bn == 256 && !prx_gemm8p_eligible(d))) { bm = 128; bn = 128; }
    else if (!want_fit && bm == 256 && bn != 256 && (d.f32 || bn == 128)) bm = 128;
    const int kt_total = ceil_div(d.K, d.f32 ? BKF : BK);
    const int tiles = ceil_div(d.M, bm) * ceil_div(d.N, bn);
    int splits = 1;
    if (ws_bytes && tiles <= n_cu / 2 && kt_total >= 16 && !(bm == 256 && bn == 256) && !fit_takes && !row) {
        splits = std::max(1, std::min(std::min((320 + tiles / 2) / tiles, kt_total / 4), 32));
        while (splits > 1 && (size_t)splits * d.M * d.N * sizeof(float) > ws_bytes) --splits;
    }
    const int forced_splits = rule && rule->splits > 0 ? rule->splits : cx.force_splits;
    if (forced_splits > 0 && ws_bytes && !fit) {
        splits = std::min(forced_splits, kt_total);
        while (splits > 1 && (size_t)splits * d.M * d.N * sizeof(float) > ws_bytes) --splits;
    }
    p->kt_per_split = ceil_div(kt_total, splits);
    if (bm == 256 && bn == 256) p->kt_per_split = (p->kt_per_split + 1) & ~1;
    p->splits = ceil_div(kt_total, p->kt_per_split);
    p->bm = bm; p->bn = bn;
    if (!row) p->family = fit ? GEMM_FIT : d.f32 ? GEMM_TILED_F32 : (bm == 256 && bn == 256) ? GEMM_8PHASE
                        : (!d.a_is_f32 && cx.use_glds) ? GEMM_TILED_GLDS : GEMM_TILED_V1;
    p->xcd_swizzle = tiles >= 16 && (cx.xcd_swizzle == 1 || (cx.xcd_swizzle == 2 && d.a_mode == PRX_A_ROWMAJOR && d.N <= 1024));
    if (cx.xcd_swizzle == 3) p->xcd_swizzle = tiles >= 16;
    if (bm == 256 && bn == 256 && cx.xcd_swizzle == 2) p->xcd_swizzle = tiles >= 512 && d.N <= 4096;
    if (fit && cx.xcd_swizzle == 2) p->xcd_swizzle = tiles >= 16;
    p->fit_flags = fit ? (cx.fit_flags & (15 | 64)) : (cx.fit_flags & 64);
    if (fit && (cx.fit_flags & 32) == 0 && d.N > d.M) p->fit_flags |= 16;
    p->stages = cx.force_stages ? cx.force_stages : ((bm == 64 && bn == 64) ? 3 : 2);
    p->c64 = d.a_mode == PRX_A_CONV3X3 && d.Cin % BK == 0 && cx.conv_c64 != 0;
}

int prx_gemm_plan_impl(const GemmDesc& d, const GemmCtx* c, int n_cu, size_t ws_bytes, bool ws_al16, GemmPlan* p) {
    static const GemmCtx k_default;
    const GemmCtx& cx = c ? *c : k_default;
    *p = GemmPlan{};
    const int v = validate(d, cx);
    if (v) return v;
    n_cu = n_cu > 0 ? n_cu : 256;
    int dbg = cx.dbg_count;
    GemmLaunchPlan& l0 = p->launch[0];
    const bool forced = cx.force_bm != 0 || find_rule(d, cx) != nullptr;
    if (!forced && cx.rowk && (long long)d.M * d.N >= cx.rowk_min && prx_gemmrow_plan(d, &l0.row_nt, &l0.row_ksm))
        l0.family = d.a_mode == PRX_A_ROWMAJOR ? GEMM_ROW : GEMM_ROWCONV;
    else if (!forced && (p->rows_8p = plan_8phase(d, cx, n_cu)) > 0)
        l0.family = GEMM_8PHASE;
    p->n_launch = p->rows_8p > 0 && p->rows_8p < d.M ? 2 : 1;
    plan_launch(p->n_launch == 2 ? rows_of(d, 0, p->rows_8p) : d, cx, n_cu, ws_bytes, ws_al16, &l0, &dbg);
    if (p->n_launch == 2) plan_launch(rows_of(d, p->rows_8p, d.M - p->rows_8p), cx, n_cu, ws_bytes, ws_al16, &p->launch[1], &dbg);
    p->dbg_used = dbg - cx.dbg_count;

    PRX_REQUIRE((d.act != PRX_ACT_GELU && d.act != PRX_ACT_MUL_DGELU) || (l0.vec_epi && !d.f32),
                "gemm: the GELU / MUL_DGELU epilogues need the vector epilogue (N %% 4 == 0, aligned operands) of the 16-bit operand kernels");
    PRX_REQUIRE(d.row16 == 0 || l0.vec_epi, "gemm: 16-bit residual / GroupNorm-input streams need the vector epilogue (N %% 4 == 0, aligned operands)");
    if (d.gnb_x) {
        PRX_REQUIRE(d.gn_stats && d.gnb_fstats && d.gnb_gamma && d.gnb_beta && (d.out_f32 || d.out_bf16) && d.act == PRX_ACT_NONE,
                    "gemm: fused GroupNorm-backward sums need gn_stats, gnb_fstats, gnb_gamma, gnb_beta and a plain output");
        PRX_REQUIRE(((uintptr_t)d.gnb_x % 16) == 0 && ((uintptr_t)d.gnb_gamma % 16) == 0 && ((uintptr_t)d.gnb_beta % 16) == 0,
                    "gemm: gnb operands must be 16-byte aligned");
    }
    p->stats_pass = d.f32 && d.gn_stats && l0.family != GEMM_FIT;
    if (p->stats_pass) {
        PRX_REQUIRE(d.out_f32 && d.ldc_f32 == d.N && d.N == 32 * d.gn_gs, "gemm: fp32 GroupNorm statistics need a dense fp32 output with N == 32 * gn_gs");
        l0 = GemmLaunchPlan{};
        plan_launch(without_stats(d), cx, n_cu, ws_bytes, ws_al16, &l0, &dbg);
        p->dbg_used = dbg - cx.dbg_count;
    } else if (d.gn_stats) {
        PRX_REQUIRE(l0.vec_epi && d.gn_gs >= 4 && d.gn_gs % 4 == 0 && d.N == 32 * d.gn_gs && !d.a_is_f32 && (cx.use_glds || d.f32),
                    "gemm: fused GroupNorm statistics need the v2 kernel's vector epilogue and N == 32 * gn_gs");
    }
    return 0;
}

static int launch_planned(const GemmDesc& d, const GemmLaunchPlan& p, float* ws, int n_cu, hipStream_t stream, GemmCtx* ctx) {
    const GemmArgs a{d, ceil_div(d.M, p.bm), ceil_div(d.N, p.bn), p.splits, p.kt_per_split, ceil_div(d.K, d.f32 ? BKF : BK), p.vec_epi,
                     p.xcd_swizzle, p.fit_flags, ws};

    GemmProfRec rec{};
    bool prof = false;
    if (ctx) {
        std::lock_guard<std::mutex> lk(ctx->mu);
        prof = ctx->prof_on;
    }
    if (prof) {
        PRX_CHECK_HIP(hipEventCreate(&rec.a));
        PRX_CHECK_HIP(hipEventCreate(&rec.b));
        const bool row = p.family == GEMM_ROW || p.family == GEMM_ROWCONV;
        rec.flop = 2.0 * d.M * d.N * d.K;
        rec.M = d.M; rec.N = d.N; rec.K = d.K; rec.mode = d.a_mode + 2 * d.up + 4 * d.a_is_f32 + 8 * d.f32;
        rec.bm = p.bm + (p.family == GEMM_FIT ? 1000 : (row ? 2000 : 0)); rec.bn = p.bn; rec.splits = p.splits;
        PRX_CHECK_HIP(hipEventRecord(rec.a, stream));
    }

    const dim3 grid(a.tiles_m * a.tiles_n, p.splits);
    const bool t128 = p.bm == 128 && p.bn == 128, t12864 = p.bm == 128 && p.bn == 64;
    const bf16_t* zp = p.family == GEMM_TILED_GLDS ? zero_page_for_current_device() : nullptr;
    PRX_REQUIRE(zp != nullptr || p.family != GEMM_TILED_GLDS, "gemm: could not allocate the zero page");
    int e = 0;
    switch (p.family) {
    case GEMM_ROW: case GEMM_ROWCONV: prx_gemmrow_launch(a, p.row_nt, p.row_ksm, n_cu, stream); break;
    case GEMM_FIT: e = prx_gemmfit_launch(a, p.bm, p.bn, grid, stream); break;
    case GEMM_8PHASE: prx_gemm8p_launch(a, grid, stream); break;
    case GEMM_TILED_F32:
        if (t128) launch_f32<128, 128>(a, grid, stream);
        else if (t12864) launch_f32<128, 64>(a, grid, stream);
        else launch_f32<64, 64>(a, grid, stream);
        break;
    case GEMM_TILED_GLDS:
        if (t128) launch_glds<128, 128>(a, grid, stream, zp, p.stages, p.c64);
        else if (t12864) launch_glds<128, 64>(a, grid, stream, zp, p.stages, p.c64);
        else launch_glds<64, 64>(a, grid, stream, zp, p.stages, p.c64);
        break;
    case GEMM_TILED_V1:
        if (t128) launch_cfg<128, 128>(a, grid, stream);
        else if (t12864) launch_cfg<128, 64>(a, grid, stream);
        else launch_cfg<64, 64>(a, grid, stream);
        break;
    }
    if (e) return e;
    PRX_LAUNCH_CHECK();
    if (p.splits > 1) {
        size_t total = (size_t)d.M * d.N;
        int blocks = (int)std::min<size_t>((total + 255) / 256, 2048);
        PRX_OP_DISPATCH(d.f32, d.h16, T, hipLaunchKernelGGL(splitk_reduce_kernel<T>, dim3(blocks), dim3(256), 0, stream, a));
        PRX_LAUNCH_CHECK();
    }
    if (prof) {
        PRX_CHECK_HIP(hipEventRecord(rec.b, stream));
        std::lock_guard<std::mutex> lk(ctx->mu);
        ctx->prof.push_back(rec);
    }
    return 0;
}

int prx_gemm_launch(const GemmDesc& d, float* ws, size_t ws_bytes, hipStream_t stream, GemmCtx* ctx) {
    int cur_dev = -1;
    if (ctx && (ctx->n_cu == 0 || (hipGetDevice(&cur_dev) == hipSuccess && cur_dev != ctx->n_cu_dev))) {
        int dev = 0, cus = 0;
        if (hipGetDevice(&dev) == hipSuccess && hipDeviceGetAttribute(&cus, hipDeviceAttributeMultiprocessorCount, dev) == hipSuccess && cus > 0)
            { ctx->n_cu = cus; ctx->n_cu_dev = dev; }
        else
            ctx->n_cu = 256;
    }
    const int n_cu = ctx && ctx->n_cu > 0 ? ctx->n_cu : 256;
    GemmPlan plan;
    const int r = prx_gemm_plan_impl(d, ctx, n_cu, ws ? ws_bytes : 0, ((uintptr_t)ws & 15) == 0, &plan);
    if (ctx) ctx->dbg_count += plan.dbg_used;
    if (r) return r;
    for (int i = 0; i < plan.n_launch; ++i) {
        const GemmDesc di = plan.n_launch == 2 ? (i == 0 ? rows_of(d, 0, plan.rows_8p) : rows_of(d, plan.rows_8p, d.M - plan.rows_8p))
                                               : (plan.stats_pass ? without_stats(d) : d);
        const int e = launch_planned(di, plan.launch[i], ws, n_cu, stream, ctx);
        if (e) return e;
    }
    if (!plan.stats_pass) return 0;
    if (d.gnb_x) return prx_groupnorm_bwd_stats(d.out_f32, d.gnb_x, d.gnb_gamma, d.gnb_beta, d.gnb_fstats, d.gn_stats, 1, d.M, d.N, d.gnb_swish, d.gnb_eps, stream);
    return prx_groupnorm_fwd(d.out_f32, nullptr, nullptr, d.gn_stats, nullptr, nullptr, 1, d.M, d.N, 0, 1e-6f, stream, 0, 0);
}
```

pixray_amd/csrc/gemm_epi.h:

```cpp
#pragma once
#include "gemm.h"
#include <type_traits>

namespace prx_gemm_dev {

struct GemmArgs {
    GemmDesc d;
    int tiles_m, tiles_n, splits, kt_per_split, kt_total;
    int vec_epi;
    int xcd_swizzle;
    int fit_flags;
    float* ws;
};

__device__ __forceinline__ float quickgelu_f(float t) { return t * sigmoidf_(1.702f * t); }
__device__ __forceinline__ float dquickgelu_f(float t) {
    float s = sigmoidf_(1.702f * t);
    return s * (1.f + 1.702f * t * (1.f - s));
}
__device__ __forceinline__ float gelu_f(float t) { return 0.5f * t * (1.f + erff(t * 0.70710678f)); }
__device__ __forceinline__ float dgelu_f(float t) {
    return 0.5f * (1.f + erff(t * 0.70710678f)) + t * (0.39894228f * __expf(-0.5f * t * t));
}

struct GnbConst { float mean, rstd; float4 ga, be; };
__device__ __forceinline__ GnbConst gnb_load(const GemmDesc& d, int col) {
    GnbConst c;
    const int g = col / d.gn_gs;
    const double n = (double)d.M * d.gn_gs;
    const double m = d.gnb_fstats[g * 2] / n;
    double var = d.gnb_fstats[g * 2 + 1] / n - m * m;
    if (var < 0) var = 0;
    c.mean = (float)m;
    c.rstd = (float)(1.0 / sqrt(var + (double)d.gnb_eps));
    c.ga = *reinterpret_cast<const float4*>(d.gnb_gamma + col);
    c.be = *reinterpret_cast<const float4*>(d.gnb_beta + col);
    return c;
}
template <typename TOp>
__device__ __forceinline__ void gnb_accum(const GemmDesc& d, const GnbConst& c, int row, int col, const float4& o, float& s0, float& s1) {
    const float4 x4 = (d.row16 & 2) ? op_ld4v(reinterpret_cast<const TOp*>(d.gnb_x), (size_t)row * d.N + col)
                                    : *reinterpret_cast<const float4*>(d.gnb_x + (size_t)row * d.N + col);
    const float xv[4] = {x4.x, x4.y, x4.z, x4.w}, gv[4] = {o.x, o.y, o.z, o.w};
    const float gav[4] = {c.ga.x, c.ga.y, c.ga.z, c.ga.w}, bev[4] = {c.be.x, c.be.y, c.be.z, c.be.w};
#pragma unroll
    for (int i = 0; i < 4; ++i) {
        const float xh = (xv[i] - c.mean) * c.rstd;
        float gy = gv[i];
        if (d.gnb_swish) {
            const float y = xh * gav[i] + bev[i];
            const float sg = sigmoidf_(y);
            gy *= sg * (1.f + y * (1.f - sg));
        }
        const float dxh = gy * gav[i];
        s0 += dxh;
        s1 += dxh * xh;
    }
}

template <typename TOp>
__device__ __forceinline__ void epilogue_store(const GemmDesc& d, int row, int col, float v) {
    const TOp* aux = reinterpret_cast<const TOp*>(d.aux);
    v *= d.alpha_dev ? d.alpha * *d.alpha_dev : d.alpha;
    if (d.bias_n) v += d.bias_n[col];
    if (d.bias_m) v += d.bias_m[row];
    if (d.act == PRX_ACT_MUL_DQUICKGELU) v *= dquickgelu_f(op_ld(aux, (size_t)row * d.ldaux + col));
    const bool masked = (d.act == PRX_ACT_MUL_RELUMASK || d.act == PRX_ACT_RELUMASK_POST) && !(op_ld(aux, (size_t)row * d.ldaux + col) > 0.f);
    if (masked && d.act == PRX_ACT_MUL_RELUMASK) v = 0.f;
    if (d.resid) v += d.resid[(size_t)row * d.ldr + col];
    if (masked && d.act == PRX_ACT_RELUMASK_POST) v = 0.f;
    if (d.act == PRX_ACT_RELU) v = fmaxf(v, 0.f);
    if (d.act == PRX_ACT_QUICKGELU) {
        const TOp pre = op_cvt<TOp>(v);
        if (d.out_bf16_pre) reinterpret_cast<TOp*>(d.out_bf16_pre)[(size_t)row * d.ldc_bf16 + col] = pre;
        v = quickgelu_f((float)pre);
    }
    if (d.out_f32) d.out_f32[(size_t)row * d.ldc_f32 + col] = v;
    if (d.out_bf16) op_st(reinterpret_cast<TOp*>(d.out_bf16), (size_t)row * d.ldc_bf16 + col, v);
}

template <typename TOp>
__device__ __forceinline__ float4 epilogue_math4(int act, float alpha, float4 v, const float4& bias, float bias_m, const float (&aux)[4],
                                                 bool has_resid, const float4& res, float4& pre) {
    v.x *= alpha; v.y *= alpha; v.z *= alpha; v.w *= alpha;
    v.x += bias.x; v.y += bias.y; v.z += bias.z; v.w += bias.w;
    v.x += bias_m; v.y += bias_m; v.z += bias_m; v.w += bias_m;
    if (act == PRX_ACT_MUL_DQUICKGELU) {
        v.x *= dquickgelu_f(aux[0]); v.y *= dquickgelu_f(aux[1]); v.z *= dquickgelu_f(aux[2]); v.w *= dquickgelu_f(aux[3]);
    }
    if (act == PRX_ACT_MUL_DGELU) {
        v.x *= dgelu_f(aux[0]); v.y *= dgelu_f(aux[1]); v.z *= dgelu_f(aux[2]); v.w *= dgelu_f(aux[3]);
    }
    const bool masked = act == PRX_ACT_MUL_RELUMASK || act == PRX_ACT_RELUMASK_POST;
    const bool k0 = !masked || aux[0] > 0.f, k1 = !masked || aux[1] > 0.f, k2 = !masked || aux[2] > 0.f, k3 = !masked || aux[3] > 0.f;
    if (act == PRX_ACT_MUL_RELUMASK) {
        if (!k0) v.x = 0.f;
// ... 92 lines not shown
```

pixray_amd/csrc/vqgan.hip:

```cpp
#include "vqgan.h"
#include "gemm.h"
#include "norms.h"
#include "elementwise.h"
#include "prompt_vq.h"
#include "vit.h"
#include "dev_arena.h"
#include <vector>
#include <memory>
#include <stdlib.h>

namespace {

template <typename TOp>
__global__ __launch_bounds__(256) void pack_conv3x3_kernel(const float* __restrict__ w, TOp* __restrict__ Wf,
                                                           TOp* __restrict__ Wd, int Cout, int Cin, int CoP) {
    const size_t total_f = (size_t)Cout * 9 * Cin;
    const size_t total_d = (size_t)Cin * 9 * CoP;
    for (size_t i = (size_t)blockIdx.x * blockDim.x + threadIdx.x; i < total_f + total_d;
         i += (size_t)gridDim.x * blockDim.x) {
        if (i < total_f) {
            int ci = (int)(i % Cin);
            int tap = (int)((i / Cin) % 9);
            int co = (int)(i / ((size_t)9 * Cin));
            Wf[i] = op_cvt<TOp>(w[(((size_t)co * Cin + ci) * 3 + tap / 3) * 3 + tap % 3]);
        } else {
            size_t j = i - total_f;
            int co = (int)(j % CoP);
            int tap = (int)((j / CoP) % 9);
            int ci = (int)(j / ((size_t)9 * CoP));
            int ky = 2 - tap / 3, kx = 2 - tap % 3;
            Wd[j] = op_cvt<TOp>((co < Cout) ? w[(((size_t)co * Cin + ci) * 3 + ky) * 3 + kx] : 0.f);
        }
    }
}

__global__ __launch_bounds__(256) void colminmax_kernel(const float* __restrict__ w, float* __restrict__ mn,
                                                        float* __restrict__ mx, int rows, int D) {
    const int c = blockIdx.x * blockDim.x + threadIdx.x;
    if (c >= D) return;
    float a = INFINITY, b = -INFINITY;
    for (int r = 0; r < rows; ++r) { float v = w[(size_t)r * D + c]; a = fminf(a, v); b = fmaxf(b, v); }
    mn[c] = a; mx[c] = b;
}

}

int prx_vqgan_pack_conv3x3(const float* w, void* Wf, void* Wd, int Cout, int Cin, int CoP, int prec, hipStream_t s) {
    PRX_REQUIRE(prec_valid(prec), "vqgan pack_conv3x3: unknown precision %d", prec);
    PRX_OP_DISPATCH(prec_is_f32(prec), prec_is_h16(prec), TO,
                    hipLaunchKernelGGL(pack_conv3x3_kernel<TO>, dim3(1024), dim3(256), 0, s, w, (TO*)Wf, (TO*)Wd, Cout, Cin, CoP));
    PRX_LAUNCH_CHECK();
    return 0;
}
int prx_colminmax(const float* w, float* mn, float* mx, int rows, int D, hipStream_t s) {
    hipLaunchKernelGGL(colminmax_kernel, dim3(ceil_div(D, 256)), dim3(256), 0, s, w, mn, mx, rows, D);
    PRX_LAUNCH_CHECK();
    return 0;
}

static inline int pad8(int P) { return (P + 7) & ~7; }

struct Conv3 { int Cin, Cout, CoP; void *Wf, *Wd; float* b; };
struct Conv1 { int Cin, Cout; void *W, *WT; float* b; };
struct GN { int C; float *g, *b; double *stats, *bstats; int id; };

struct ResBlock {
    int Cin, Cout, rh, rw;
    GN n1, n2; Conv3 c1, c2; Conv1 sc; bool has_sc;
    void *x_in, *h1, *scbuf, *out;
    void *x_in_bf, *out_bf;
};
struct AttnBlock {
    int C, rh, rw;
    GN n; Conv1 qkv, proj;
    void* x_in; void *qkvb, *Pm, *PT; void* out; void* out_bf;
    void* qkvT;
};
struct UpBlock { int C, rh, rw; Conv3 c; void *x_in, *out; void *x_in_bf, *out_bf; };

struct Stage { int kind; int idx; };

struct PrxVqgan {
    int zc, D, NC, ch, out_ch, h0, w0, H, W, nstage;
    int prec;
    int f32, h16;
    int lean;
    float* gs;
    GemmCtx gctx;
    DevArena mem;
    float *codebook, *cnorm, *zmin, *zmax;
    Conv1 pq; Conv3 conv_in, conv_out; GN norm_out;
    std::vector<ResBlock> res; std::vector<AttnBlock> attn; std::vector<UpBlock> ups; std::vector<Stage> stages;
    float *zq, *y, *dzq; void* h_in; int* idx; void *pqo_bf, *h_in_bf, *dpq_bf;
    float *pmin; int* pidx;
    void* a;
    void *tA, *tB, *tC, *tD, *dqkv, *dy8;
    void *dycol, *Wd_col;
    float* S;
    void *g0, *g1, *g2;
    void *g0b, *g1b, *g2b;
    double* all_stats; int n_gn;
    float* ws; size_t ws_bytes;
    void* x_last;
};

namespace {
int alloc_stream(PrxVqgan* v, void** p, size_t count) { return v->mem.alloc_op(p, count, !v->lean); }

struct WCursor { const float* const* w; int n, pos; };
#define NEXTW(cur, dst) do { PRX_REQUIRE((cur).pos < (cur).n, "vqgan_create: weight list too short"); (dst) = (cur).w[(cur).pos++]; } while (0)

int make_gn(PrxVqgan* v, GN& g, int C, WCursor& cur, hipStream_t s) {
    const float *w, *b; NEXTW(cur, w); NEXTW(cur, b);
    g.C = C;
    int r;
    if ((r = v->mem.copy_f32(&g.g, w, C, s))) return r;
    if ((r = v->mem.copy_f32(&g.b, b, C, s))) return r;
    g.id = v->n_gn++;
    g.stats = g.bstats = nullptr;
    return 0;
}
int make_conv3(PrxVqgan* v, Conv3& c, int Cin, int Cout, WCursor& cur, hipStream_t s) {
    const float *w, *b; NEXTW(cur, w); NEXTW(cur, b);
    c.Cin = Cin; c.Cout = Cout; c.CoP = (Cout + 7) / 8 * 8;
    DEV_ALLOC(v->mem, alloc_op, c.Wf, (size_t)c.CoP * 9 * Cin, v->f32);
    if (c.CoP != Cout) PRX_CHECK_HIP(hipMemsetAsync(c.Wf, 0, (size_t)c.CoP * 9 * Cin * op_esz(v->f32), s));
    DEV_ALLOC(v->mem, alloc_op, c.Wd, (size_t)Cin * 9 * c.CoP, v->f32);
    { int e_ = prx_vqgan_pack_conv3x3(w, c.Wf, c.Wd, Cout, Cin, c.CoP, v->prec, s); if (e_) return e_; }
    DEV_ALLOC(v->mem, alloc, c.b, c.CoP);
    if (c.CoP != Cout) PRX_CHECK_HIP(hipMemsetAsync(c.b, 0, sizeof(float) * c.CoP, s));
    PRX_CHECK_HIP(hipMemcpyAsync(c.b, b, sizeof(float) * Cout, hipMemcpyDeviceToDevice, s));
    return 0;
}
int make_conv1(PrxVqgan* v, Conv1& c, int Cin, int Cout, WCursor& cur, hipStream_t s) {
    const float *w, *b; NEXTW(cur, w); NEXTW(cur, b);
    c.Cin = Cin; c.Cout = Cout;
    DEV_ALLOC(v->mem, alloc_op, c.W, (size_t)Cout * Cin, v->f32); DEV_ALLOC(v->mem, alloc_op, c.WT, (size_t)Cout * Cin, v->f32);
    int r;
    if ((r = prx_pack_op(w, c.W, (size_t)Cout * Cin, v->prec, s))) return r;
    if ((r = prx_pack_transpose_op(w, c.WT, Cout, Cin, v->prec, s))) return r;
    return v->mem.copy_f32(&c.b, b, Cout, s);
}
int make_res(PrxVqgan* v, int Cin, int Cout, int rh, int rw, WCursor& cur, hipStream_t s) {
    ResBlock rb{};
    rb.Cin = Cin; rb.Cout = Cout; rb.rh = rh; rb.rw = rw; rb.has_sc = Cin != Cout;
    int r;
    if ((r = make_gn(v, rb.n1, Cin, cur, s))) return r;
    if ((r = make_conv3(v, rb.c1, Cin, Cout, cur, s))) return r;
    if ((r = make_gn(v, rb.n2, Cout, cur, s))) return r;
    if ((r = make_conv3(v, rb.c2, Cout, Cout, cur, s))) return r;
    const size_t P = (size_t)rh * rw;
    if (rb.has_sc) {
        if ((r = make_conv1(v, rb.sc, Cin, Cout, cur, s))) return r;
        if ((r = alloc_stream(v, &rb.scbuf, P * Cout))) return r;
    }
    if ((r = alloc_stream(v, &rb.h1, P * Cout))) return r;
    if ((r = alloc_stream(v, &rb.out, P * Cout))) return r;
    v->stages.push_back({0, (int)v->res.size()});
    v->res.push_back(rb);
    return 0;
}
int make_attn(PrxVqgan* v, int C, int rh, int rw, WCursor& cur, hipStream_t s) {
    AttnBlock ab{};
    ab.C = C; ab.rh = rh; ab.rw = rw;
    int r;
    if ((r = make_gn(v, ab.n, C, cur, s))) return r;
    const float *wq, *bq, *wk, *bk, *wv, *bv;
    NEXTW(cur, wq); NEXTW(cur, bq); NEXTW(cur, wk); NEXTW(cur, bk); NEXTW(cur, wv); NEXTW(cur, bv);
    float *wcat, *bcat;
    DEV_ALLOC(v->mem, alloc, wcat, (size_t)3 * C * C); DEV_ALLOC(v->mem, alloc, bcat, 3 * C);
    const float* ws_[3] = {wq, wk, wv}; const float* bs_[3] = {bq, bk, bv};
    for (int i = 0; i < 3; ++i) {
        PRX_CHECK_HIP(hipMemcpyAsync(wcat + (size_t)i * C * C, ws_[i], sizeof(float) * C * C, hipMemcpyDeviceToDevice, s));
        PRX_CHECK_HIP(hipMemcpyAsync(bcat + i * C, bs_[i], sizeof(float) * C, hipMemcpyDeviceToDevice, s));
    }
    ab.qkv.Cin = C; ab.qkv.Cout = 3 * C; ab.qkv.b = bcat;
    DEV_ALLOC(v->mem, alloc_op, ab.qkv.W, (size_t)3 * C * C, v->f32); DEV_ALLOC(v->mem, alloc_op, ab.qkv.WT, (size_t)3 * C * C, v->f32);
    if ((r = prx_pack_op(wcat, ab.qkv.W, (size_t)3 * C * C, v->prec, s))) return r;
    if ((r = prx_pack_transpose_op(wcat, ab.qkv.WT, 3 * C, C, v->prec, s))) return r;
    if ((r = make_conv1(v, ab.proj, C, C, cur, s))) return r;
    const size_t P = (size_t)rh * rw;
    const size_t P8 = (size_t)pad8((int)P);
    DEV_ALLOC(v->mem, alloc_op, ab.qkvb, P * 3 * C, v->f32);
    DEV_ALLOC(v->mem, alloc_op, ab.Pm, P * P8, v->f32); DEV_ALLOC(v->mem, alloc_op, ab.PT, P * P8, v->f32);
    if ((r = alloc_stream(v, &ab.out, P * C))) return r;
    DEV_ALLOC(v->mem, alloc_op, ab.qkvT, (size_t)3 * C * P8, v->f32);
    PRX_CHECK_HIP(hipMemsetAsync(ab.qkvT, 0, (size_t)3 * C * P8 * op_esz(v->f32), s));
    PRX_CHECK_HIP(hipMemsetAsync(ab.Pm, 0, P * P8 * op_esz(v->f32), s));
    PRX_CHECK_HIP(hipMemsetAsync(ab.PT, 0, P * P8 * op_esz(v->f32), s));
    v->stages.push_back({1, (int)v->attn.size()});
    v->attn.push_back(ab);
    return 0;
}
int make_up(PrxVqgan* v, int C, int rh, int rw, WCursor& cur, hipStream_t s) {
    UpBlock ub{};
    ub.C = C; ub.rh = rh; ub.rw = rw;
    int r;
    if ((r = make_conv3(v, ub.c, C, C, cur, s))) return r;
    if ((r = alloc_stream(v, &ub.out, (size_t)rh * rw * C))) return r;
    v->stages.push_back({2, (int)v->ups.size()});
    v->ups.push_back(ub);
    return 0;
}
}

int prx_vqgan_create_impl(PrxVqgan** out, int ch, const int* ch_mult, int n_mult, int num_res_blocks, int attn_res,
                          int resolution, int z_channels, int embed_dim, int n_embed, int out_ch, int h0, int w0,
                          int precision, const float* const* w, int n_w, hipStream_t s) {
    PRX_REQUIRE(h0 >= 1 && w0 >= 1, "vqgan_create: bad latent size %dx%d", h0, w0);
    PRX_REQUIRE(prec_valid(precision), "vqgan_create: unknown precision %d", precision);
    PRX_REQUIRE(embed_dim == z_channels, "vqgan_create: embed_dim must equal z_channels");
    std::unique_ptr<PrxVqgan> guard(new PrxVqgan());
    PrxVqgan* v = guard.get();
    DevArena& m = v->mem;
    const int f32 = prec_is_f32(precision);
    m.describe("vqgan_create", ": the decoder keeps one forward's activations and the backward's gradient streams for a %d x %d latent", h0, w0);
    v->prec = precision; v->f32 = prec_is_f32(precision); v->h16 = prec_is_h16(precision);
    v->gs = nullptr;
    { const char* e = getenv("PRX_LEAN"); v->lean = (v->h16 && !(e && atoi(e) == 0)) ? 1 : 0; }
    v->n_gn = 0; v->zc = z_channels; v->D = embed_dim; v->NC = n_embed; v->ch = ch; v->out_ch = out_ch; v->h0 = h0; v->w0 = w0;
    WCursor cur{w, n_w, 0};
    int r;
    const float* cb; NEXTW(cur, cb);
    if ((r = m.copy_f32(&v->codebook, cb, (size_t)n_embed * embed_dim, s))) return r;
    DEV_ALLOC(m, alloc, v->cnorm, n_embed); DEV_ALLOC(m, alloc, v->zmin, embed_dim); DEV_ALLOC(m, alloc, v->zmax, embed_dim);
    if ((r = prx_sqnorm_rows(v->codebook, v->cnorm, n_embed, embed_dim, s))) return r;
    if ((r = prx_colminmax(v->codebook, v->zmin, v->zmax, n_embed, embed_dim, s))) return r;
    if ((r = make_conv1(v, v->pq, embed_dim, z_channels, cur, s))) return r;
    int block_in = ch * ch_mult[n_mult - 1];
    int rh = h0, rw = w0;
    if ((r = make_conv3(v, v->conv_in, z_channels, block_in, cur, s))) return r;
    if ((r = make_res(v, block_in, block_in, rh, rw, cur, s))) return r;
    if ((r = make_attn(v, block_in, rh, rw, cur, s))) return r;
    if ((r = make_res(v, block_in, block_in, rh, rw, cur, s))) return r;
    int nominal = resolution >> (n_mult - 1);
    for (int lvl = n_mult - 1; lvl >= 0; --lvl) {
        int block_out = ch * ch_mult[lvl];
        for (int b = 0; b < num_res_blocks + 1; ++b) {
            if ((r = make_res(v, block_in, block_out, rh, rw, cur, s))) return r;
            block_in = block_out;
            if (nominal == attn_res) { if ((r = make_attn(v, block_in, rh, rw, cur, s))) return r; }
        }
        if (lvl != 0) {
            rh *= 2; rw *= 2; nominal *= 2;
            if ((r = make_up(v, block_in, rh, rw, cur, s))) return r;
        }
    }
    v->H = rh; v->W = rw;
    if ((r = make_gn(v, v->norm_out, block_in, cur, s))) return r;
    if ((r = make_conv3(v, v->conv_out, block_in, out_ch, cur, s))) return r;
    PRX_REQUIRE(cur.pos == n_w, "vqgan_create: %d weight tensors given, %d consumed", n_w, cur.pos);
    const size_t P0 = (size_t)h0 * w0, PH = (size_t)rh * rw;
    size_t maxPC = P0 * (size_t)std::max(z_channels, embed_dim), maxAttnPC = 1;
    for (auto& rb : v->res) maxPC = std::max(maxPC, (size_t)rb.rh * rb.rw * std::max(rb.Cin, rb.Cout));
    for (auto& ub : v->ups) maxPC = std::max(maxPC, (size_t)ub.rh * ub.rw * ub.C);
    for (auto& ab : v->attn) maxAttnPC = std::max(maxAttnPC, (size_t)pad8(ab.rh * ab.rw) * (size_t)std::max(ab.C, pad8(ab.rh * ab.rw)));
    DEV_ALLOC(m, alloc, v->zq, P0 * embed_dim); DEV_ALLOC(m, alloc_op, v->pqo_bf, P0 * z_channels, f32);
    DEV_ALLOC(m, alloc_op, v->dpq_bf, P0 * z_channels, f32);
    if ((r = alloc_stream(v, &v->h_in, P0 * (size_t)(ch * ch_mult[n_mult - 1])))) return r;
    DEV_ALLOC(m, alloc, v->y, PH * (size_t)v->conv_out.CoP); DEV_ALLOC(m, alloc, v->idx, P0); DEV_ALLOC(m, alloc, v->dzq, P0 * embed_dim);
    const int ntiles = ceil_div(n_embed, 64);
    DEV_ALLOC(m, alloc, v->pmin, P0 * ntiles); DEV_ALLOC(m, alloc, v->pidx, P0 * ntiles);
    DEV_ALLOC(m, alloc_op, v->a, maxPC, f32);
    DEV_ALLOC(m, alloc_op, v->tA, maxAttnPC, f32); DEV_ALLOC(m, alloc_op, v->tB, maxAttnPC, f32); DEV_ALLOC(m, alloc_op, v->tC, maxAttnPC, f32);
    DEV_ALLOC(m, alloc_op, v->tD, maxAttnPC, f32);
    DEV_ALLOC(m, alloc_op, v->dqkv, maxAttnPC * 3, f32); DEV_ALLOC(m, alloc_op, v->dy8, PH * 8, f32);
    v->dycol = v->Wd_col = nullptr;
    if (!v->f32 && v->conv_out.CoP == 8) {
        const int Cin = v->conv_out.Cin;
        DEV_ALLOC(m, alloc_op, v->dycol, PH * 128, f32); DEV_ALLOC(m, alloc_op, v->Wd_col, (size_t)Cin * 128, f32);
        PRX_CHECK_HIP(hipMemsetAsync(v->Wd_col, 0, (size_t)Cin * 128 * sizeof(bf16_t), s));
        PRX_CHECK_HIP(hipMemcpy2DAsync(v->Wd_col, 128 * sizeof(bf16_t), v->conv_out.Wd, 72 * sizeof(bf16_t), 72 * sizeof(bf16_t), Cin, hipMemcpyDeviceToDevice, s));
    }
    DEV_ALLOC(m, alloc, v->S, maxAttnPC);
    for (void** g : {&v->g0, &v->g1, &v->g2})
        if ((r = alloc_stream(v, g, maxPC))) return r;
    if (v->f32 || v->lean) { v->g0b = v->g0; v->g1b = v->g1; v->g2b = v->g2; }
    else { DEV_ALLOC(m, alloc_op, v->g0b, maxPC, f32); DEV_ALLOC(m, alloc_op, v->g1b, maxPC, f32); DEV_ALLOC(m, alloc_op, v->g2b, maxPC, f32); }
    v->h_in_bf = nullptr;
    for (size_t i = 0; i < v->stages.size(); ++i) {
        const Stage& st = v->stages[i];
        const bool need = (st.kind == 0 && v->res[st.idx].has_sc) || st.kind == 2;
        if (!need) continue;
        void** slot; size_t cnt; void* self;
        if (i == 0) { slot = &v->h_in_bf; cnt = P0 * (size_t)(ch * ch_mult[n_mult - 1]); self = v->h_in; }
        else {
            const Stage& pr = v->stages[i - 1];
            if (pr.kind == 0) { ResBlock& b = v->res[pr.idx]; slot = &b.out_bf; cnt = (size_t)b.rh * b.rw * b.Cout; self = b.out; }
            else if (pr.kind == 1) { AttnBlock& b = v->attn[pr.idx]; slot = &b.out_bf; cnt = (size_t)b.rh * b.rw * b.C; self = b.out; }
            else { UpBlock& b = v->ups[pr.idx]; slot = &b.out_bf; cnt = (size_t)b.rh * b.rw * b.C; self = b.out; }
        }
        if (v->f32 || v->lean) *slot = self;
        else DEV_ALLOC(m, alloc_op, *slot, cnt, f32);
    }
    {
        DEV_ALLOC(m, alloc, v->all_stats, (size_t)2 * v->n_gn * 64);
        auto fix = [&](GN& g) { g.stats = v->all_stats + (size_t)g.id * 64; g.bstats = v->all_stats + (size_t)(v->n_gn + g.id) * 64; };
        for (auto& b : v->res) { fix(b.n1); fix(b.n2); }
        for (auto& b : v->attn) fix(b.n);
        fix(v->norm_out);
    }
    v->ws_bytes = (size_t)64 << 20;
    DEV_ALLOC(m, alloc, v->ws, v->ws_bytes / sizeof(float));
    if (v->h16) DEV_ALLOC(m, alloc, v->gs, 2 + 256);
    *out = guard.release();
    return 0;
}

void prx_vqgan_destroy_impl(PrxVqgan* v) { delete v; }

static bool fusable(const PrxVqgan* v, int C) {
    static const bool f32_fuse = [] { const char* e = getenv("PRX_F32_GN_FUSE"); return !(e && atoi(e) == 0); }();
    const int gs = C / 32;
    return (!v->f32 || f32_fuse) && C % 32 == 0 && gs >= 4 && (gs & (gs - 1)) == 0;
}

static int zero_if_padded(const PrxVqgan* v, void* buf, size_t rows, int P, hipStream_t s) {
    if (pad8(P) != P) PRX_CHECK_HIP(hipMemsetAsync(buf, 0, rows * (size_t)pad8(P) * op_esz(v->f32), s));
    return 0;
}


static void vq_trace(const PrxVqgan* v, const char* tag, int i, const void* p_, size_t n, hipStream_t s) {
    static const bool on = getenv("PRX_VQ_TRACE") != nullptr;
    if (!on || !p_ || v->lean) return;
    const float* p = (const float*)p_;
    std::vector<float> h(n);
    (void)hipStreamSynchronize(s);
    (void)hipMemcpy(h.data(), p, n * sizeof(float), hipMemcpyDeviceToHost);
    double q = 0, mx = 0;
    for (float x : h) { q += (double)x * x; mx = fabs(x) > mx ? fabs(x) : mx; }
    fprintf(stderr, "[vq] %s %2d n=%zu l2 %.9e max %.6e\n", tag, i, n, sqrt(q), mx);
}

static int vg(PrxVqgan* v, GemmDesc& d, hipStream_t s) {
    if (v->f32) {
        d.f32 = 1; d.a_is_f32 = 0;
        if (d.out_bf16 == (void*)d.out_f32) d.out_bf16 = nullptr;
    }
    d.h16 = v->h16;
    return prx_gemm_launch(d, v->ws, v->ws_bytes, s, &v->gctx);
}
GemmCtx* prx_vqgan_gemm_ctx_impl(PrxVqgan* v) { return v ? &v->gctx : nullptr; }

static void out_stream(const PrxVqgan* v, GemmDesc& d, void* stream, int ld, void* twin) {
    if (v->lean) { d.out_bf16 = stream ? stream : twin; d.ldc_bf16 = ld; }
    else { d.out_f32 = (float*)stream; d.ldc_f32 = ld; d.out_bf16 = twin; d.ldc_bf16 = ld; }
}
static void resid_stream(const PrxVqgan* v, GemmDesc& d, const void* r, int ld) {
    if (!r) return;
    d.ldr = ld;
    d.resid = (const float*)r;
    if (v->lean) d.row16 |= 1;
}
static int conv3_fwd(PrxVqgan* v, const Conv3& c, const void* x, bool x_f32, int rh, int rw, bool up, const void* resid,
                     void* out, int ldc, hipStream_t s, void* out_bf = nullptr, const GN* stats_for = nullptr, bool f32_out = false) {
    GemmDesc d; d.A = x; d.a_is_f32 = x_f32; d.a_mode = PRX_A_CONV3X3; d.lda = c.Cin;
    d.B = c.Wf; d.ldb = 9 * c.Cin; d.M = rh * rw; d.N = c.CoP; d.K = 9 * c.Cin;
    d.H = rh; d.W = rw; d.Cin = c.Cin; d.up = up; d.bias_n = c.b;
    resid_stream(v, d, resid, c.Cout);
    if (f32_out) { d.out_f32 = (float*)out; d.ldc_f32 = ldc; }
    else { out_stream(v, d, out, ldc, out_bf); if (!v->lean) d.ldc_bf16 = c.Cout; }
    if (stats_for && stats_for->C == c.Cout && fusable(v, c.Cout)) { d.gn_stats = stats_for->stats; d.gn_gs = c.Cout / 32; }
    return vg(v, d, s);
}
static void set_gnb(const PrxVqgan* v, GemmDesc& d, const GN* gnb, const void* gnb_x, int swish) {
    if (!gnb || !fusable(v, gnb->C) || d.N != gnb->C) return;
    d.gn_stats = gnb->bstats; d.gn_gs = gnb->C / 32;
    d.gnb_x = (const float*)gnb_x;
    if (v->lean) d.row16 |= 2;
    d.gnb_fstats = gnb->stats; d.gnb_gamma = gnb->g; d.gnb_beta = gnb->b; d.gnb_swish = swish; d.gnb_eps = 1e-6f;
}
static int conv3_bwd(PrxVqgan* v, const Conv3& c, const void* dy, bool dy_f32, int rh, int rw, void* dx, hipStream_t s,
                     void* dx_bf = nullptr, const GN* gnb = nullptr, const void* gnb_x = nullptr, int gnb_swish = 1) {
    GemmDesc d; d.A = dy; d.a_is_f32 = dy_f32; d.a_mode = PRX_A_CONV3X3; d.lda = c.CoP;
    d.B = c.Wd; d.ldb = 9 * c.CoP; d.M = rh * rw; d.N = c.Cin; d.K = 9 * c.CoP;
    d.H = rh; d.W = rw; d.Cin = c.CoP; d.up = 0;
    out_stream(v, d, dx, c.Cin, dx_bf);
    set_gnb(v, d, gnb, gnb_x, gnb_swish);
    return vg(v, d, s);
}
static const GN* first_norm(const PrxVqgan* v, int si) {
    if (si >= (int)v->stages.size()) return &v->norm_out;
    const Stage& st = v->stages[si];
    if (st.kind == 0) return &v->res[st.idx].n1;
    if (st.kind == 1) return &v->attn[st.idx].n;
    return nullptr;
}
static int gn_fwd(PrxVqgan* v, const GN& g, const void* x, int P, int swish, hipStream_t s, bool stats_ready = false) {
    return prx_groupnorm_fwd(x, g.g, g.b, g.stats, v->f32 ? nullptr : (bf16_t*)v->a, v->f32 ? (float*)v->a : nullptr, 1, P, g.C, swish,
                             1e-6f, s, 0, stats_ready ? 1 : 0, v->h16, v->lean);
}
static int gn_bwd(PrxVqgan* v, const GN& g, const void* grad, const void* x, const void* add, void* dx,
                  void* dx_bf, int P, int swish, hipStream_t s, bool stats_ready = false) {
    return prx_groupnorm_bwd(grad, x, g.g, g.b, g.stats, g.bstats, add, v->lean ? nullptr : (float*)dx, v->f32 ? nullptr : (bf16_t*)dx_bf, 1, P, g.C,
                             swish, 1e-6f, s, 0, stats_ready && fusable(v, g.C) ? 1 : 0, v->h16, v->lean);
}

int prx_vqgan_bounds_impl(PrxVqgan* v, float* zmin, float* zmax, hipStream_t s) {
    PRX_CHECK_HIP(hipMemcpyAsync(zmin, v->zmin, sizeof(float) * v->D, hipMemcpyDeviceToDevice, s));
    PRX_CHECK_HIP(hipMemcpyAsync(zmax, v->zmax, sizeof(float) * v->D, hipMemcpyDeviceToDevice, s));
    return 0;
}

int prx_vqgan_synth_impl(PrxVqgan* v, const float* z, float* img, int* indices, int quantize, hipStream_t s) {
    const int P0 = v->h0 * v->w0;
    int r;
    PRX_CHECK_HIP(hipMemsetAsync(v->all_stats, 0, sizeof(double) * (size_t)v->n_gn * 64, s));
    if (quantize) {
        if ((r = prx_vq_nearest(z, 1, P0, v->codebook, v->cnorm, P0, v->NC, v->D, v->pmin, v->pidx, v->idx, v->zq, s))) return r;
        if (indices) PRX_CHECK_HIP(hipMemcpyAsync(indices, v->idx, sizeof(int) * P0, hipMemcpyDeviceToDevice, s));
    } else {
        if ((r = prx_nchw_to_nhwc(z, v->zq, nullptr, 1, v->zc, P0, v->zc, s))) return r;
    }
    {   GemmDesc d; d.A = v->zq; d.a_is_f32 = 1; d.lda = v->D; d.B = v->pq.W; d.ldb = v->D; d.M = P0; d.N = v->zc; d.K = v->D;
        d.bias_n = v->pq.b; d.out_bf16 = v->pqo_bf; d.ldc_bf16 = v->zc;
        if ((r = vg(v, d, s))) return r; }
    const GN* nx = first_norm(v, 0);
    if ((r = conv3_fwd(v, v->conv_in, v->pqo_bf, false, v->h0, v->w0, false, nullptr, v->h_in, v->conv_in.Cout, s, v->h_in_bf, nx))) return r;
    bool sr = nx && nx->C == v->conv_in.Cout && fusable(v, nx->C);
    void* x = v->h_in;
    void* x_bf = v->h_in_bf;
    for (int si = 0; si < (int)v->stages.size(); ++si) {
        const Stage& st = v->stages[si];
        nx = first_norm(v, si + 1);
        if (st.kind == 0) {
            ResBlock& b = v->res[st.idx];
            const int P = b.rh * b.rw;
            b.x_in = x; b.x_in_bf = x_bf;
            if ((r = gn_fwd(v, b.n1, x, P, 1, s, sr))) return r;
            if ((r = conv3_fwd(v, b.c1, v->a, false, b.rh, b.rw, false, nullptr, b.h1, b.Cout, s, nullptr, &b.n2))) return r;
            const void* resid = x;
            if (b.has_sc) {
                PRX_REQUIRE(x_bf != nullptr, "vqgan: missing bf16 twin for the shortcut input");
                GemmDesc d; d.A = x_bf; d.lda = b.Cin; d.B = b.sc.W; d.ldb = b.Cin; d.M = P; d.N = b.Cout; d.K = b.Cin;
                d.bias_n = b.sc.b; out_stream(v, d, b.scbuf, b.Cout, nullptr);
                if ((r = vg(v, d, s))) return r;
                resid = b.scbuf;
            }
            if ((r = gn_fwd(v, b.n2, b.h1, P, 1, s, fusable(v, b.Cout)))) return r;
            if ((r = conv3_fwd(v, b.c2, v->a, false, b.rh, b.rw, false, resid, b.out, b.Cout, s, b.out_bf, nx))) return r;
            sr = nx && nx->C == b.Cout && fusable(v, b.Cout);
            x = b.out; x_bf = b.out_bf;
        } else if (st.kind == 1) {
            AttnBlock& b = v->attn[st.idx];
            const int P = b.rh * b.rw, C = b.C;
            b.x_in = x;
            if ((r = gn_fwd(v, b.n, x, P, 0, s, sr))) return r;
            {   GemmDesc d; d.A = v->a; d.lda = C; d.B = b.qkv.W; d.ldb = C; d.M = P; d.N = 3 * C; d.K = C;
                d.bias_n = b.qkv.b; d.out_bf16 = b.qkvb; d.ldc_bf16 = 3 * C;
                if ((r = vg(v, d, s))) return r; }
            const int P8 = pad8(P);
            if ((r = prx_transpose_op(b.qkvb, 3 * C, b.qkvT, P8, P, 3 * C, v->f32, s))) return r;
            {   GemmDesc d; d.A = b.qkvb; d.lda = 3 * C; d.B = op_off(b.qkvb, C, v->f32); d.ldb = 3 * C; d.M = P; d.N = P; d.K = C;
                d.out_f32 = v->S; d.ldc_f32 = P;
                if ((r = vg(v, d, s))) return r; }
            if ((r = prx_softmax_rows(v->S, P, 1.f / sqrtf((float)C), b.Pm, P8, b.PT, P8, P, P, v->prec, s))) return r;
            {   GemmDesc d; d.A = b.Pm; d.lda = P8; d.B = op_off(b.qkvT, (size_t)2 * C * P8, v->f32); d.ldb = P8; d.M = P; d.N = C; d.K = P8;
                d.out_bf16 = v->tB; d.ldc_bf16 = C;
                if ((r = vg(v, d, s))) return r; }
            {   GemmDesc d; d.A = v->tB; d.lda = C; d.B = b.proj.W; d.ldb = C; d.M = P; d.N = C; d.K = C;
                d.bias_n = b.proj.b; resid_stream(v, d, x, C); out_stream(v, d, b.out, C, b.out_bf);
                if (nx && nx->C == C && fusable(v, C)) { d.gn_stats = nx->stats; d.gn_gs = C / 32; }
                if ((r = vg(v, d, s))) return r; }
            sr = nx && nx->C == C && fusable(v, C);
            x = b.out; x_bf = b.out_bf;
        } else {
            UpBlock& b = v->ups[st.idx];
            b.x_in = x; b.x_in_bf = x_bf;
            PRX_REQUIRE(x_bf != nullptr, "vqgan: missing bf16 twin for the upsample input");
            if ((r = conv3_fwd(v, b.c, x_bf, false, b.rh, b.rw, true, nullptr, b.out, b.C, s, b.out_bf, nx))) return r;
            sr = nx && nx->C == b.C && fusable(v, b.C);
            x = b.out; x_bf = b.out_bf;
        }
        {   const int Pq = st.kind == 0 ? v->res[st.idx].rh * v->res[st.idx].rw : st.kind == 1 ? v->attn[st.idx].rh * v->attn[st.idx].rw : v->ups[st.idx].rh * v->ups[st.idx].rw;
            const int Cq = st.kind == 0 ? v->res[st.idx].Cout : st.kind == 1 ? v->attn[st.idx].C : v->ups[st.idx].C;
            vq_trace(v, "fwd", si, x, (size_t)Pq * Cq, s); }
    }
    v->x_last = x;
    const int PH = v->H * v->W;
    if ((r = gn_fwd(v, v->norm_out, x, PH, 1, s, sr))) return r;
    if ((r = conv3_fwd(v, v->conv_out, v->a, false, v->H, v->W, false, nullptr, v->y, v->conv_out.CoP, s, nullptr, nullptr, true))) return r;
    return prx_image_head_fwd(v->y, v->conv_out.CoP, img, 1, v->out_ch, PH, s);
}

long long prx_vqgan_debug_stage_impl(PrxVqgan* v, int stage, float* dst, long long max_floats, hipStream_t s) {
    const void* src = nullptr; long long n = 0;
    PRX_REQUIRE(!v->lean || stage == -2 || stage >= (int)v->stages.size(), "vqgan debug_stage: the stage outputs are 16-bit in the lean layout (PRX_LEAN=0 for fp32 streams)");
    const int ns = (int)v->stages.size();
    if (stage == -2) { src = v->zq; n = (long long)v->h0 * v->w0 * v->D; }
    else if (stage == -1) { src = v->h_in; n = (long long)v->h0 * v->w0 * v->conv_in.Cout; }
    else if (stage >= 0 && stage < ns) {
        const Stage& st = v->stages[stage];
        if (st.kind == 0) { const ResBlock& b = v->res[st.idx]; src = b.out; n = (long long)b.rh * b.rw * b.Cout; }
        else if (st.kind == 1) { const AttnBlock& b = v->attn[st.idx]; src = b.out; n = (long long)b.rh * b.rw * b.C; }
        else { const UpBlock& b = v->ups[st.idx]; src = b.out; n = (long long)b.rh * b.rw * b.C; }
    } else if (stage == ns) { src = v->y; n = (long long)v->H * v->W * v->conv_out.CoP; }
    else if (stage == ns + 1) { src = reinterpret_cast<const float*>(v->all_stats); n = (long long)v->n_gn * 64 * 2; }
    else return -1;
    if (n > max_floats) n = max_floats;
    if (hipMemcpyAsync(dst, src, sizeof(float) * n, hipMemcpyDeviceToDevice, s) != hipSuccess) return -1;
    return n;
}

int prx_vqgan_backward_impl(PrxVqgan* v, const float* g_img, float* dz, hipStream_t s) {
    const int PH = v->H * v->W;
    int r;
    PRX_REQUIRE(v->x_last != nullptr, "vqgan backward: no forward in flight on this handle");
    PRX_CHECK_HIP(hipMemsetAsync(v->all_stats + (size_t)v->n_gn * 64, 0, sizeof(double) * (size_t)v->n_gn * 64, s));
    if (v->h16 && (r = prx_grad_scale(g_img, (size_t)v->out_ch * PH, v->gs + 2, 256, prx_grad_target_log2(), v->gs, s))) return r;
    struct GB { void* f; void* b; };
    GB g{v->g0, v->g0b}, t1{v->g1, v->g1b}, t2{v->g2, v->g2b};
    if (v->dycol) {
        if ((r = prx_image_head_bwd_im2col(v->y, v->conv_out.CoP, g_img, (bf16_t*)v->dycol, 128, v->out_ch, v->H, v->W, s, v->h16, v->gs))) return r;
        GemmDesc d; d.A = v->dycol; d.lda = 128; d.B = v->Wd_col; d.ldb = 128; d.M = PH; d.N = v->conv_out.Cin; d.K = 128;
        out_stream(v, d, t1.f, v->conv_out.Cin, nullptr);
        set_gnb(v, d, &v->norm_out, v->x_last, 1);
        if ((r = vg(v, d, s))) return r;
    } else {
        if ((r = prx_image_head_bwd(v->y, v->conv_out.CoP, g_img, v->f32 ? (float*)v->dy8 : nullptr, v->f32 ? nullptr : (bf16_t*)v->dy8, v->conv_out.CoP, 1,
                                    v->out_ch, PH, s, v->h16, v->gs))) return r;
        if ((r = conv3_bwd(v, v->conv_out, v->dy8, false, v->H, v->W, t1.f, s, nullptr, &v->norm_out, v->x_last, 1))) return r;
    }
    if ((r = gn_bwd(v, v->norm_out, t1.f, v->x_last, nullptr, g.f, g.b, PH, 1, s, true))) return r;
    for (int si = (int)v->stages.size() - 1; si >= 0; --si) {
        const Stage& st = v->stages[si];
        if (st.kind == 0) {
            ResBlock& b = v->res[st.idx];
            const int P = b.rh * b.rw;
            if ((r = conv3_bwd(v, b.c2, g.b, false, b.rh, b.rw, t1.f, s, nullptr, &b.n2, b.h1, 1))) return r;
            if ((r = gn_bwd(v, b.n2, t1.f, b.h1, nullptr, v->f32 ? t2.f : nullptr, t2.b, P, 1, s, true))) return r;
            if ((r = conv3_bwd(v, b.c1, t2.b, false, b.rh, b.rw, t1.f, s, nullptr, &b.n1, b.x_in, 1))) return r;
            const void* add = g.f;
            if (b.has_sc) {
                GemmDesc d; d.A = g.b; d.lda = b.Cout; d.B = b.sc.WT; d.ldb = b.Cout; d.M = P; d.N = b.Cin; d.K = b.Cout;
                out_stream(v, d, t2.f, b.Cin, nullptr);
                if ((r = vg(v, d, s))) return r;
                add = t2.f;
            }
            GB& dst = (add == g.f) ? t2 : g;
            if ((r = gn_bwd(v, b.n1, t1.f, b.x_in, add, dst.f, dst.b, P, 1, s, true))) return r;
            if (&dst != &g) std::swap(g, t2);
        } else if (st.kind == 1) {
            AttnBlock& b = v->attn[st.idx];
            const int P = b.rh * b.rw, C = b.C;
            {   GemmDesc d; d.A = g.b; d.lda = C; d.B = b.proj.WT; d.ldb = C; d.M = P; d.N = C; d.K = C;
                d.out_bf16 = v->tA; d.ldc_bf16 = C;
                if ((r = vg(v, d, s))) return r; }
            {   GemmDesc d; d.A = v->tA; d.lda = C; d.B = op_off(b.qkvb, 2 * C, v->f32); d.ldb = 3 * C; d.M = P; d.N = P; d.K = C;
                d.out_f32 = v->S; d.ldc_f32 = P;
                if ((r = vg(v, d, s))) return r; }
            const int P8 = pad8(P);
            if ((r = zero_if_padded(v, v->tB, P, P, s))) return r;
            if ((r = zero_if_padded(v, v->tC, P, P, s))) return r;
            if ((r = prx_softmax_rows_bwd(b.Pm, P8, v->S, P, 1.f / sqrtf((float)C), v->tB, P8, v->tC, P8, P, P, v->prec, s))) return r;
            {   GemmDesc d; d.A = v->tB; d.lda = P8; d.B = op_off(b.qkvT, (size_t)C * P8, v->f32); d.ldb = P8; d.M = P; d.N = C; d.K = P8;
                d.out_bf16 = v->dqkv; d.ldc_bf16 = 3 * C;
                if ((r = vg(v, d, s))) return r; }
            {   GemmDesc d; d.A = v->tC; d.lda = P8; d.B = b.qkvT; d.ldb = P8; d.M = P; d.N = C; d.K = P8;
                d.out_bf16 = op_off(v->dqkv, C, v->f32); d.ldc_bf16 = 3 * C;
                if ((r = vg(v, d, s))) return r; }
            if ((r = zero_if_padded(v, v->tD, C, P, s))) return r;
            if ((r = prx_transpose_op(v->tA, C, v->tD, P8, P, C, v->f32, s))) return r;
            {   GemmDesc d; d.A = b.PT; d.lda = P8; d.B = v->tD; d.ldb = P8; d.M = P; d.N = C; d.K = P8;
                d.out_bf16 = op_off(v->dqkv, 2 * C, v->f32); d.ldc_bf16 = 3 * C;
                if ((r = vg(v, d, s))) return r; }
            {   GemmDesc d; d.A = v->dqkv; d.lda = 3 * C; d.B = b.qkv.WT; d.ldb = 3 * C; d.M = P; d.N = C; d.K = 3 * C;
                out_stream(v, d, t1.f, C, nullptr);
                set_gnb(v, d, &b.n, b.x_in, 0);
                if ((r = vg(v, d, s))) return r; }
            if ((r = gn_bwd(v, b.n, t1.f, b.x_in, g.f, t2.f, t2.b, P, 0, s, true))) return r;
            std::swap(g, t2);
        } else {
            UpBlock& b = v->ups[st.idx];
            if ((r = conv3_bwd(v, b.c, g.b, false, b.rh, b.rw, t1.f, s))) return r;
            if ((r = prx_upsample2x_bwd(t1.f, v->lean ? nullptr : (float*)t2.f, v->f32 ? nullptr : (bf16_t*)t2.b, 1, b.rh / 2, b.rw / 2, b.C, s, v->h16,
                                        v->lean))) return r;
            std::swap(g, t2);
        }
        {   const int Pq = st.kind == 0 ? v->res[st.idx].rh * v->res[st.idx].rw : st.kind == 1 ? v->attn[st.idx].rh * v->attn[st.idx].rw : v->ups[st.idx].rh * v->ups[st.idx].rw / 4;
            const int Cq = st.kind == 0 ? v->res[st.idx].Cin : st.kind == 1 ? v->attn[st.idx].C : v->ups[st.idx].C;
            vq_trace(v, "bwd", si, g.f, (size_t)Pq * Cq, s); }
    }
    if ((r = conv3_bwd(v, v->conv_in, g.b, false, v->h0, v->w0, v->lean ? nullptr : t1.f, s, v->dpq_bf))) return r;
    const int P0 = v->h0 * v->w0;
    {   GemmDesc d; d.A = v->dpq_bf; d.lda = v->zc; d.B = v->pq.WT; d.ldb = v->zc; d.M = P0; d.N = v->D; d.K = v->zc;
        d.out_f32 = v->dzq; d.ldc_f32 = v->D;
        if (v->h16) d.alpha_dev = v->gs + 1;
        if ((r = vg(v, d, s))) return r; }
    return prx_nhwc_to_nchw(v->dzq, v->D, dz, 1, v->D, P0, s);
}
```

Before: 169.6.

## Fuse VQGAN attention transposes into softmax kernels and group backward attention GEMMs

Folds the qkv transpose into the forward softmax launch and the tA transpose into the backward softmax launch by appending transpose tiles to the grid. It also batches the three backward dQ/dK/dV GEMMs into one grouped launch using blockIdx.z, falling back to separate launches when the plans differ. The aim is fewer kernel launches and more parallel work per launch in the small-spatial attention blocks. This adds kernel specialisation and a per-member operand select, and the grouped path only applies when all three GEMMs get identical plans.

```diff
diff --git a/include/prx.h b/include/prx.h
--- a/include/prx.h
+++ b/include/prx.h
@@ -62,6 +62,8 @@
                   prx_stream_t stream);
 long long prx_gemm_fit_spec_launches(void);
 long long prx_gemm_row_launches(void);
+int prx_k_gemm_group(const prx_gemm_args* g, int n, void* ws, size_t ws_bytes, prx_stream_t stream);
+long long prx_gemm_group_launches(void);
 
 int prx_k_groupnorm_fwd(const float* x, const float* gamma, const float* beta, double* stats, void* out_bf16,
                         float* out_f32, int NB, int P, int C, int swish, float eps, prx_stream_t s);
@@ -123,6 +125,11 @@
                           int prec, prx_stream_t s);
 int prx_k_softmax_rows_bwd_op(const void* P, int ldp, const float* dP, int lddp, float scale, void* dS, int ldds, void* dST,
                               int lddst, int rows, int cols, int prec, prx_stream_t s);
+int prx_k_softmax_rows_tr_op(const float* S, int lds_, float scale, void* P, int ldp, void* PT, int ldpt, int rows, int cols,
+                             const void* tin, int ldtin, void* tout, int ldtout, int tR, int tC, int prec, prx_stream_t s);
+int prx_k_softmax_rows_bwd_tr_op(const void* P, int ldp, const float* dP, int lddp, float scale, void* dS, int ldds, void* dST,
+                                 int lddst, int rows, int cols, const void* tin, int ldtin, void* tout, int ldtout, int tR, int tC,
+                                 int prec, prx_stream_t s);
 int prx_k_transpose_op(const void* in, int ldin, void* out, int ldout, int R, int C, int f32, prx_stream_t s);
 int prx_k_upsample2x_bwd_op(const void* hi, float* low, void* low16, int NB, int Hl, int Wl, int C, int h16, int s16,
                             prx_stream_t s);
diff --git a/pixray_amd/csrc/api_core.hip b/pixray_amd/csrc/api_core.hip
--- a/pixray_amd/csrc/api_core.hip
+++ b/pixray_amd/csrc/api_core.hip
@@ -73,6 +73,17 @@
     if (r) return r;
     return prx_gemm_launch(d, (float*)ws, ws_bytes, (hipStream_t)stream_, (GemmCtx*)g->ctx);
 }
+int prx_k_gemm_group(const prx_gemm_args* g, int n, void* ws, size_t ws_bytes, prx_stream_t stream_) {
+    PRX_REQUIRE(g != nullptr && n >= 1 && n <= 4, "prx_k_gemm_group: 1 to 4 members (got %d)", n);
+    GemmDesc d[4];
+    for (int i = 0; i < n; ++i) {
+        const int r = desc_of(g + i, d[i]);
+        if (r) return r;
+        PRX_REQUIRE(g[i].ctx == g[0].ctx, "prx_k_gemm_group: the members must share one context");
+    }
+    return prx_gemm_launch_group(d, n, (float*)ws, ws_bytes, (hipStream_t)stream_, (GemmCtx*)g[0].ctx);
+}
+long long prx_gemm_group_launches(void) { return prx_gemm_group_launches_impl(); }
 int prx_k_gemm_gn(const prx_gemm_args* g, double* gn_stats, int gn_gs, const float* gnb_x, const double* gnb_fstats,
                   const float* gnb_gamma, const float* gnb_beta, int gnb_swish, float gnb_eps, void* ws, size_t ws_bytes,
                   prx_stream_t stream_) {
diff --git a/pixray_amd/csrc/api_kernels.hip b/pixray_amd/csrc/api_kernels.hip
--- a/pixray_amd/csrc/api_kernels.hip
+++ b/pixray_amd/csrc/api_kernels.hip
@@ -207,6 +207,17 @@
     PRX_REQUIRE(prec_valid(prec), "softmax_rows_bwd: unknown precision %d", prec);
     return prx_softmax_rows_bwd(P, ldp, dP, lddp, scale, dS, ldds, dST, lddst, rows, cols, prec, S_(s));
 }
+int prx_k_softmax_rows_tr_op(const float* S, int lds_, float scale, void* P, int ldp, void* PT, int ldpt, int rows, int cols,
+                             const void* tin, int ldtin, void* tout, int ldtout, int tR, int tC, int prec, prx_stream_t s) {
+    PRX_REQUIRE(prec_valid(prec), "softmax_rows_tr: unknown precision %d", prec);
+    return prx_softmax_rows_tr(S, lds_, scale, P, ldp, PT, ldpt, rows, cols, tin, ldtin, tout, ldtout, tR, tC, prec, S_(s));
+}
+int prx_k_softmax_rows_bwd_tr_op(const void* P, int ldp, const float* dP, int lddp, float scale, void* dS, int ldds, void* dST,
+                                 int lddst, int rows, int cols, const void* tin, int ldtin, void* tout, int ldtout, int tR, int tC,
+                                 int prec, prx_stream_t s) {
+    PRX_REQUIRE(prec_valid(prec), "softmax_rows_bwd_tr: unknown precision %d", prec);
+    return prx_softmax_rows_bwd_tr(P, ldp, dP, lddp, scale, dS, ldds, dST, lddst, rows, cols, tin, ldtin, tout, ldtout, tR, tC, prec, S_(s));
+}
 int prx_k_transpose_op(const void* in, int ldin, void* out, int ldout, int R, int C, int f32, prx_stream_t s) {
     return prx_transpose_op(in, ldin, out, ldout, R, C, f32, S_(s));
 }
diff --git a/pixray_amd/csrc/elementwise.h b/pixray_amd/csrc/elementwise.h
--- a/pixray_amd/csrc/elementwise.h
+++ b/pixray_amd/csrc/elementwise.h
@@ -5,6 +5,10 @@
                      int cols, int prec, hipStream_t s);
 int prx_softmax_rows_bwd(const void* P, int ldp, const float* dP, int lddp, float scale, void* dS, int ldds,
                          void* dST, int lddst, int rows, int cols, int prec, hipStream_t s);
+int prx_softmax_rows_tr(const float* S, int lds_, float scale, void* P, int ldp, void* PT, int ldpt, int rows, int cols,
+                        const void* tin, int ldtin, void* tout, int ldtout, int tR, int tC, int prec, hipStream_t s);
+int prx_softmax_rows_bwd_tr(const void* P, int ldp, const float* dP, int lddp, float scale, void* dS, int ldds, void* dST, int lddst,
+                            int rows, int cols, const void* tin, int ldtin, void* tout, int ldtout, int tR, int tC, int prec, hipStream_t s);
 int prx_upsample2x_bwd(const void* hi, float* low, bf16_t* low_bf16, int NB, int Hl, int Wl, int C, hipStream_t s, int h16 = 0, int s16 = 0);
 int prx_nchw_to_nhwc(const float* in, float* out_f32, bf16_t* out_bf16, int NB, int C, int HW, int Cpad, hipStream_t s, int h16 = 0);
 int prx_nhwc_to_nchw(const float* in, int ldc, float* out, int NB, int C, int HW, hipStream_t s);
diff --git a/pixray_amd/csrc/elementwise.hip b/pixray_amd/csrc/elementwise.hip
--- a/pixray_amd/csrc/elementwise.hip
+++ b/pixray_amd/csrc/elementwise.hip
@@ -6,11 +6,11 @@
 inline int ew_grid(size_t total, int per = 256) { return (int)std::min<size_t>((total + per - 1) / per, 8192); }
 
 template <typename T>
-__global__ __launch_bounds__(256) void transpose_op_kernel(const T* __restrict__ in, int ldin,
-                                                           T* __restrict__ out, int ldout, int R, int C) {
+__device__ __forceinline__ void transpose_op_tile(const T* __restrict__ in, int ldin, T* __restrict__ out, int ldout, int R, int C,
+                                                  int bx, int by) {
     __shared__ T tile[32][33];
     const int tx = threadIdx.x & 31, ty = threadIdx.x >> 5;
-    const int r0 = blockIdx.y * 32, c0 = blockIdx.x * 32;
+    const int r0 = by * 32, c0 = bx * 32;
 #pragma unroll
     for (int i = 0; i < 4; ++i) {
         int r = r0 + ty + 8 * i, c = c0 + tx;
@@ -23,13 +23,17 @@
         if (c < C && r < R) out[(size_t)c * ldout + r] = tile[tx][ty + 8 * i];
     }
 }
-
-template <typename T>
-__global__ __launch_bounds__(256) void softmax_rows_kernel(const float* __restrict__ S, int lds_, float scale,
-                                                           T* __restrict__ P, int ldp, T* __restrict__ PT,
-                                                           int ldpt, int rows, int cols) {
+template <typename T>
+__global__ __launch_bounds__(256) void transpose_op_kernel(const T* __restrict__ in, int ldin,
+                                                           T* __restrict__ out, int ldout, int R, int C) {
+    transpose_op_tile<T>(in, ldin, out, ldout, R, C, blockIdx.x, blockIdx.y);
+}
+
+template <typename T>
+__device__ __forceinline__ void softmax_rows_body(const float* __restrict__ S, int lds_, float scale, T* __restrict__ P, int ldp,
+                                                  T* __restrict__ PT, int ldpt, int rows, int cols, int blk) {
     const int lane = threadIdx.x & 63;
-    const int row = blockIdx.x * 4 + (threadIdx.x >> 6);
+    const int row = blk * 4 + (threadIdx.x >> 6);
     if (row >= rows) return;
     const float* s = S + (size_t)row * lds_;
     float mx = -INFINITY;
@@ -45,14 +49,19 @@
         if (PT) PT[(size_t)c * ldpt + row] = p;
     }
 }
-
-template <typename T>
-__global__ __launch_bounds__(256) void softmax_rows_bwd_kernel(const T* __restrict__ P, int ldp,
-                                                               const float* __restrict__ dP, int lddp, float scale,
-                                                               T* __restrict__ dS, int ldds,
-                                                               T* __restrict__ dST, int lddst, int rows, int cols) {
+template <typename T>
+__global__ __launch_bounds__(256) void softmax_rows_kernel(const float* __restrict__ S, int lds_, float scale,
+                                                           T* __restrict__ P, int ldp, T* __restrict__ PT,
+                                                           int ldpt, int rows, int cols) {
+    softmax_rows_body<T>(S, lds_, scale, P, ldp, PT, ldpt, rows, cols, blockIdx.x);
+}
+
+template <typename T>
+__device__ __forceinline__ void softmax_rows_bwd_body(const T* __restrict__ P, int ldp, const float* __restrict__ dP, int lddp, float scale,
+                                                      T* __restrict__ dS, int ldds, T* __restrict__ dST, int lddst, int rows, int cols,
+                                                      int blk) {
     const int lane = threadIdx.x & 63;
-    const int row = blockIdx.x * 4 + (threadIdx.x >> 6);
+    const int row = blk * 4 + (threadIdx.x >> 6);
     if (row >= rows) return;
     float dot = 0.f;
     for (int c = lane; c < cols; c += 64)
@@ -64,6 +73,32 @@
         dS[(size_t)row * ldds + c] = v;
         if (dST) dST[(size_t)c * lddst + row] = v;
     }
+}
+template <typename T>
+__global__ __launch_bounds__(256) void softmax_rows_bwd_kernel(const T* __restrict__ P, int ldp,
+                                                               const float* __restrict__ dP, int lddp, float scale,
+                                                               T* __restrict__ dS, int ldds,
+                                                               T* __restrict__ dST, int lddst, int rows, int cols) {
+    softmax_rows_bwd_body<T>(P, ldp, dP, lddp, scale, dS, ldds, dST, lddst, rows, cols, blockIdx.x);
+}
+
+struct TransposeRider { const void* in; int ldin; void* out; int ldout, R, C, tiles_c; };
+template <typename T, typename TT>
+__global__ __launch_bounds__(256) void softmax_rows_tr_kernel(const float* __restrict__ S, int lds_, float scale, T* __restrict__ P, int ldp,
+                                                              T* __restrict__ PT, int ldpt, int rows, int cols, const TransposeRider tr) {
+    const int nsoft = (rows + 3) >> 2;
+    if ((int)blockIdx.x < nsoft) { softmax_rows_body<T>(S, lds_, scale, P, ldp, PT, ldpt, rows, cols, blockIdx.x); return; }
+    const int t = (int)blockIdx.x - nsoft, by = t / tr.tiles_c;
+    transpose_op_tile<TT>((const TT*)tr.in, tr.ldin, (TT*)tr.out, tr.ldout, tr.R, tr.C, t - by * tr.tiles_c, by);
+}
+template <typename T, typename TT>
+__global__ __launch_bounds__(256) void softmax_rows_bwd_tr_kernel(const T* __restrict__ P, int ldp, const float* __restrict__ dP, int lddp,
+                                                                  float scale, T* __restrict__ dS, int ldds, T* __restrict__ dST, int lddst,
+                                                                  int rows, int cols, const TransposeRider tr) {
+    const int nsoft = (rows + 3) >> 2;
+    if ((int)blockIdx.x < nsoft) { softmax_rows_bwd_body<T>(P, ldp, dP, lddp, scale, dS, ldds, dST, lddst, rows, cols, blockIdx.x); return; }
+    const int t = (int)blockIdx.x - nsoft, by = t / tr.tiles_c;
+    transpose_op_tile<TT>((const TT*)tr.in, tr.ldin, (TT*)tr.out, tr.ldout, tr.R, tr.C, t - by * tr.tiles_c, by);
 }
 
 template <bool S16>
@@ -294,6 +329,37 @@
     PRX_LAUNCH_CHECK();
     return 0;
 }
+int prx_softmax_rows_tr(const float* S, int lds_, float scale, void* P, int ldp, void* PT, int ldpt, int rows, int cols,
+                        const void* tin, int ldtin, void* tout, int ldtout, int tR, int tC, int prec, hipStream_t s) {
+    PRX_REQUIRE(rows > 0 && tR > 0 && tC > 0 && tin && tout, "softmax_rows_tr: empty softmax or transpose");
+    const TransposeRider tr{tin, ldtin, tout, ldtout, tR, tC, ceil_div(tC, 32)};
+    const dim3 grid(ceil_div(rows, 4) + tr.tiles_c * ceil_div(tR, 32));
+    if (prec_is_f32(prec))
+        hipLaunchKernelGGL((softmax_rows_tr_kernel<float, float>), grid, dim3(256), 0, s, S, lds_, scale, (float*)P, ldp, (float*)PT, ldpt, rows, cols, tr);
+    else if (prec_is_h16(prec))
+        hipLaunchKernelGGL((softmax_rows_tr_kernel<half_t, bf16_t>), grid, dim3(256), 0, s, S, lds_, scale, (half_t*)P, ldp, (half_t*)PT, ldpt, rows, cols, tr);
+    else
+        hipLaunchKernelGGL((softmax_rows_tr_kernel<bf16_t, bf16_t>), grid, dim3(256), 0, s, S, lds_, scale, (bf16_t*)P, ldp, (bf16_t*)PT, ldpt, rows, cols, tr);
+    PRX_LAUNCH_CHECK();
+    return 0;
+}
+int prx_softmax_rows_bwd_tr(const void* P, int ldp, const float* dP, int lddp, float scale, void* dS, int ldds, void* dST, int lddst,
+                            int rows, int cols, const void* tin, int ldtin, void* tout, int ldtout, int tR, int tC, int prec, hipStream_t s) {
+    PRX_REQUIRE(rows > 0 && tR > 0 && tC > 0 && tin && tout, "softmax_rows_bwd_tr: empty softmax or transpose");
+    const TransposeRider tr{tin, ldtin, tout, ldtout, tR, tC, ceil_div(tC, 32)};
+    const dim3 grid(ceil_div(rows, 4) + tr.tiles_c * ceil_div(tR, 32));
+    if (prec_is_f32(prec))
+        hipLaunchKernelGGL((softmax_rows_bwd_tr_kernel<float, float>), grid, dim3(256), 0, s, (const float*)P, ldp, dP, lddp, scale, (float*)dS, ldds,
+                           (float*)dST, lddst, rows, cols, tr);
+    else if (prec_is_h16(prec))
+        hipLaunchKernelGGL((softmax_rows_bwd_tr_kernel<half_t, bf16_t>), grid, dim3(256), 0, s, (const half_t*)P, ldp, dP, lddp, scale, (half_t*)dS, ldds,
+                           (half_t*)dST, lddst, rows, cols, tr);
+    else
+        hipLaunchKernelGGL((softmax_rows_bwd_tr_kernel<bf16_t, bf16_t>), grid, dim3(256), 0, s, (const bf16_t*)P, ldp, dP, lddp, scale, (bf16_t*)dS, ldds,
+                           (bf16_t*)dST, lddst, rows, cols, tr);
+    PRX_LAUNCH_CHECK();
+    return 0;
+}
 int prx_upsample2x_bwd(const void* hi, float* low, bf16_t* low_bf16, int NB, int Hl, int Wl, int C, hipStream_t s, int h16, int s16) {
     PRX_REQUIRE(C % 4 == 0 && (low || low_bf16), "upsample2x_bwd: C %% 4 != 0, or no output");
     if (s16) hipLaunchKernelGGL(upsample2x_bwd_kernel<true>, dim3(ew_grid((size_t)NB * Hl * Wl * C / 4)), dim3(256), 0, s, hi, low, low_bf16,
diff --git a/pixray_amd/csrc/gemm.h b/pixray_amd/csrc/gemm.h
--- a/pixray_amd/csrc/gemm.h
+++ b/pixray_amd/csrc/gemm.h
@@ -97,3 +97,6 @@
 int prx_gemm_ctx_profile_collect(GemmCtx* c, double* total_ms, double* total_flop, long long* launches);
 
 int prx_gemm_launch(const GemmDesc& d, float* ws, size_t ws_bytes, hipStream_t stream, GemmCtx* ctx = nullptr);
+
+int prx_gemm_launch_group(const GemmDesc* d, int n, float* ws, size_t ws_bytes, hipStream_t stream, GemmCtx* ctx = nullptr);
+long long prx_gemm_group_launches_impl();
diff --git a/pixray_amd/csrc/gemm.hip b/pixray_amd/csrc/gemm.hip
--- a/pixray_amd/csrc/gemm.hip
+++ b/pixray_amd/csrc/gemm.hip
@@ -2,6 +2,7 @@
 #include "norms.h"
 #include <vector>
 #include <mutex>
+#include <atomic>
 #include <stdlib.h>
 #include <type_traits>
 
@@ -372,8 +373,8 @@
 typedef const __attribute__((address_space(1))) void* gptr_t;
 typedef __attribute__((address_space(3))) void* lptr_t;
 
-template <int BM, int BN, int AMODE, int STAGES, bool C64 = false, int NWM = 2, typename T16 = bf16_t>
-__global__ __launch_bounds__(NWM * 128) void gemm_glds_kernel(const GemmArgs p, const bf16_t* __restrict__ zero_page) {
+template <int BM, int BN, int AMODE, int STAGES, bool C64 = false, int NWM = 2, typename T16 = bf16_t, int GROUP = 0>
+__global__ __launch_bounds__(NWM * 128) void gemm_glds_kernel(const GemmArgs p, const bf16_t* __restrict__ zero_page, const GemmGroupArg<GROUP> grp) {
     constexpr int NW = NWM * 2;
     constexpr int A_IN = BM / (8 * NW);
     constexpr int B_IN = BN / (8 * NW);
@@ -384,7 +385,16 @@
 
     __shared__ __attribute__((aligned(16))) bf16_t lds[STAGES * TILE];
 
-    const GemmDesc& d = p.d;
+    GemmDesc dg;
+    if constexpr (GROUP != 0) {
+        const int g = blockIdx.z;
+        dg = p.d;
+        dg.A = g == 0 ? grp.A[0] : g == 1 ? grp.A[1] : g == 2 ? grp.A[2] : grp.A[3];
+        dg.B = g == 0 ? grp.B[0] : g == 1 ? grp.B[1] : g == 2 ? grp.B[2] : grp.B[3];
+        dg.out_f32 = g == 0 ? grp.out_f32[0] : g == 1 ? grp.out_f32[1] : g == 2 ? grp.out_f32[2] : grp.out_f32[3];
+        dg.out_bf16 = g == 0 ? grp.out_bf16[0] : g == 1 ? grp.out_bf16[1] : g == 2 ? grp.out_bf16[2] : grp.out_bf16[3];
+    }
+    const GemmDesc& d = GROUP != 0 ? dg : p.d;
     const int tid = threadIdx.x;
     const int lane = tid & 63;
     const int wave = __builtin_amdgcn_readfirstlane(tid >> 6);
@@ -770,11 +780,11 @@
 template <int BM, int BN, int STAGES, typename T16>
 void launch_glds_t(const GemmArgs& a, dim3 grid, hipStream_t s, const bf16_t* zero_page, bool c64) {
     if (a.d.a_mode == PRX_A_ROWMAJOR)
-        hipLaunchKernelGGL((gemm_glds_kernel<BM, BN, PRX_A_ROWMAJOR, STAGES, false, 2, T16>), grid, dim3(256), 0, s, a, zero_page);
+        hipLaunchKernelGGL((gemm_glds_kernel<BM, BN, PRX_A_ROWMAJOR, STAGES, false, 2, T16>), grid, dim3(256), 0, s, a, zero_page, GemmGroupArg<0>{});
     else if (c64)
-        hipLaunchKernelGGL((gemm_glds_kernel<BM, BN, PRX_A_CONV3X3, STAGES, true, 2, T16>), grid, dim3(256), 0, s, a, zero_page);
+        hipLaunchKernelGGL((gemm_glds_kernel<BM, BN, PRX_A_CONV3X3, STAGES, true, 2, T16>), grid, dim3(256), 0, s, a, zero_page, GemmGroupArg<0>{});
     else
-        hipLaunchKernelGGL((gemm_glds_kernel<BM, BN, PRX_A_CONV3X3, STAGES, false, 2, T16>), grid, dim3(256), 0, s, a, zero_page);
+        hipLaunchKernelGGL((gemm_glds_kernel<BM, BN, PRX_A_CONV3X3, STAGES, false, 2, T16>), grid, dim3(256), 0, s, a, zero_page, GemmGroupArg<0>{});
 }
 template <int BM, int BN, int STAGES>
 void launch_glds_s(const GemmArgs& a, dim3 grid, hipStream_t s, const bf16_t* zero_page, bool c64) {
@@ -786,6 +796,14 @@
     if (stages >= 4 && (BM + BN) * BK * 2 * 4 <= 160 * 1024) launch_glds_s<BM, BN, 4>(a, grid, s, zero_page, c64);
     else if (stages >= 3) launch_glds_s<BM, BN, 3>(a, grid, s, zero_page, c64);
     else launch_glds_s<BM, BN, 2>(a, grid, s, zero_page, c64);
+}
+
+inline bool glds_group_stages(int bm, int bn, int stages) { return stages == ((bm == 64 && bn == 64) ? 3 : 2); }
+template <int BM, int BN>
+void launch_glds_group(const GemmArgs& a, dim3 grid, hipStream_t s, const bf16_t* zero_page, const GemmGroupArg<1>& grp) {
+    constexpr int ST = (BM == 64 && BN == 64) ? 3 : 2;
+    if (a.d.h16) hipLaunchKernelGGL((gemm_glds_kernel<BM, BN, PRX_A_ROWMAJOR, ST, false, 2, half_t, 1>), grid, dim3(256), 0, s, a, zero_page, grp);
+    else         hipLaunchKernelGGL((gemm_glds_kernel<BM, BN, PRX_A_ROWMAJOR, ST, false, 2, bf16_t, 1>), grid, dim3(256), 0, s, a, zero_page, grp);
 }
 
 std::mutex g_zero_mu;
@@ -1067,7 +1085,8 @@
     return 0;
 }
 
-static int launch_planned(const GemmDesc& d, const GemmLaunchPlan& p, float* ws, int n_cu, hipStream_t stream, GemmCtx* ctx) {
+static int launch_planned(const GemmDesc& d, const GemmLaunchPlan& p, float* ws, int n_cu, hipStream_t stream, GemmCtx* ctx,
+                          const GemmGroupArg<1>* grp = nullptr, int n_grp = 1) {
     const GemmArgs a{d, ceil_div(d.M, p.bm), ceil_div(d.N, p.bn), p.splits, p.kt_per_split, ceil_div(d.K, d.f32 ? BKF : BK), p.vec_epi,
                      p.xcd_swizzle, p.fit_flags, ws};
 
@@ -1081,13 +1100,13 @@
         PRX_CHECK_HIP(hipEventCreate(&rec.a));
         PRX_CHECK_HIP(hipEventCreate(&rec.b));
         const bool row = p.family == GEMM_ROW || p.family == GEMM_ROWCONV;
-        rec.flop = 2.0 * d.M * d.N * d.K;
+        rec.flop = 2.0 * d.M * d.N * d.K * n_grp;
         rec.M = d.M; rec.N = d.N; rec.K = d.K; rec.mode = d.a_mode + 2 * d.up + 4 * d.a_is_f32 + 8 * d.f32;
         rec.bm = p.bm + (p.family == GEMM_FIT ? 1000 : (row ? 2000 : 0)); rec.bn = p.bn; rec.splits = p.splits;
         PRX_CHECK_HIP(hipEventRecord(rec.a, stream));
     }
 
-    const dim3 grid(a.tiles_m * a.tiles_n, p.splits);
+    const dim3 grid(a.tiles_m * a.tiles_n, p.splits, grp ? n_grp : 1);
     const bool t128 = p.bm == 128 && p.bn == 128, t12864 = p.bm == 128 && p.bn == 64;
     const bf16_t* zp = p.family == GEMM_TILED_GLDS ? zero_page_for_current_device() : nullptr;
     PRX_REQUIRE(zp != nullptr || p.family != GEMM_TILED_GLDS, "gemm: could not allocate the zero page");
@@ -1102,7 +1121,12 @@
         else launch_f32<64, 64>(a, grid, stream);
         break;
     case GEMM_TILED_GLDS:
-        if (t128) launch_glds<128, 128>(a, grid, stream, zp, p.stages, p.c64);
+        if (grp) {
+            if (t128) launch_glds_group<128, 128>(a, grid, stream, zp, *grp);
+            else if (t12864) launch_glds_group<128, 64>(a, grid, stream, zp, *grp);
+            else launch_glds_group<64, 64>(a, grid, stream, zp, *grp);
+        }
+        else if (t128) launch_glds<128, 128>(a, grid, stream, zp, p.stages, p.c64);
         else if (t12864) launch_glds<128, 64>(a, grid, stream, zp, p.stages, p.c64);
         else launch_glds<64, 64>(a, grid, stream, zp, p.stages, p.c64);
         break;
@@ -1128,7 +1152,7 @@
     return 0;
 }
 
-int prx_gemm_launch(const GemmDesc& d, float* ws, size_t ws_bytes, hipStream_t stream, GemmCtx* ctx) {
+static int launch_n_cu(GemmCtx* ctx) {
     int cur_dev = -1;
     if (ctx && (ctx->n_cu == 0 || (hipGetDevice(&cur_dev) == hipSuccess && cur_dev != ctx->n_cu_dev))) {
         int dev = 0, cus = 0;
@@ -1137,7 +1161,11 @@
         else
             ctx->n_cu = 256;
     }
-    const int n_cu = ctx && ctx->n_cu > 0 ? ctx->n_cu : 256;
+    return ctx && ctx->n_cu > 0 ? ctx->n_cu : 256;
+}
+
+int prx_gemm_launch(const GemmDesc& d, float* ws, size_t ws_bytes, hipStream_t stream, GemmCtx* ctx) {
+    const int n_cu = launch_n_cu(ctx);
     GemmPlan plan;
     const int r = prx_gemm_plan_impl(d, ctx, n_cu, ws ? ws_bytes : 0, ((uintptr_t)ws & 15) == 0, &plan);
     if (ctx) ctx->dbg_count += plan.dbg_used;
@@ -1152,3 +1180,50 @@
     if (d.gnb_x) return prx_groupnorm_bwd_stats(d.out_f32, d.gnb_x, d.gnb_gamma, d.gnb_beta, d.gnb_fstats, d.gn_stats, 1, d.M, d.N, d.gnb_swish, d.gnb_eps, stream);
     return prx_groupnorm_fwd(d.out_f32, nullptr, nullptr, d.gn_stats, nullptr, nullptr, 1, d.M, d.N, 0, 1e-6f, stream, 0, 0);
 }
+
+namespace { std::atomic<long long> g_group_launches{0}; }
+long long prx_gemm_group_launches_impl() { return g_group_launches.load(std::memory_order_relaxed); }
+
+static bool same_but_operands(const GemmDesc& a, const GemmDesc& b) {
+    return a.f32 == b.f32 && a.h16 == b.h16 && a.a_is_f32 == b.a_is_f32 && a.a_mode == b.a_mode && a.lda == b.lda && a.ldb == b.ldb &&
+           a.M == b.M && a.N == b.N && a.K == b.K && a.H == b.H && a.W == b.W && a.Cin == b.Cin && a.up == b.up &&
+           a.alpha == b.alpha && a.alpha_dev == b.alpha_dev && a.bias_n == b.bias_n && a.bias_m == b.bias_m && a.aux == b.aux && a.ldaux == b.ldaux &&
+           a.resid == b.resid && a.ldr == b.ldr && a.act == b.act && a.ldc_f32 == b.ldc_f32 && a.out_bf16_pre == b.out_bf16_pre &&
+           a.ldc_bf16 == b.ldc_bf16 && a.gn_stats == b.gn_stats && a.gn_gs == b.gn_gs && a.gnb_x == b.gnb_x && a.gnb_fstats == b.gnb_fstats &&
+           a.gnb_gamma == b.gnb_gamma && a.gnb_beta == b.gnb_beta && a.gnb_swish == b.gnb_swish && a.row16 == b.row16 && a.gnb_eps == b.gnb_eps &&
+           (a.out_f32 == nullptr) == (b.out_f32 == nullptr) && (a.out_bf16 == nullptr) == (b.out_bf16 == nullptr);
+}
+static bool same_launch(const GemmLaunchPlan& a, const GemmLaunchPlan& b) {
+    return a.family == b.family && a.bm == b.bm && a.bn == b.bn && a.splits == b.splits && a.kt_per_split == b.kt_per_split &&
+           a.stages == b.stages && a.c64 == b.c64 && a.vec_epi == b.vec_epi && a.xcd_swizzle == b.xcd_swizzle && a.fit_flags == b.fit_flags;
+}
+
+int prx_gemm_launch_group(const GemmDesc* d, int n, float* ws, size_t ws_bytes, hipStream_t stream, GemmCtx* ctx) {
+    PRX_REQUIRE(d != nullptr && n >= 1 && n <= GEMM_GROUP_MAX, "gemm group: 1 to %d members (got %d)", GEMM_GROUP_MAX, n);
+    const int n_cu = launch_n_cu(ctx);
+    GemmPlan plan;
+    bool grouped = true;
+    for (int i = 0; i < n && grouped; ++i) {
+        GemmPlan pi;
+        const int r = prx_gemm_plan_impl(d[i], ctx, n_cu, ws ? ws_bytes : 0, ((uintptr_t)ws & 15) == 0, &pi);
+        if (r) return r;
+        if (i == 0) plan = pi;
+        grouped = same_but_operands(d[0], d[i]) && pi.n_launch == 1 && !pi.stats_pass && pi.dbg_used == 0 && same_launch(plan.launch[0], pi.launch[0]);
+    }
+    const GemmLaunchPlan& l0 = plan.launch[0];
+    grouped = grouped && l0.family == GEMM_TILED_GLDS && l0.splits == 1 && d[0].a_mode == PRX_A_ROWMAJOR && d[0].gn_stats == nullptr &&
+              fourwave_tile(l0.bm, l0.bn) && glds_group_stages(l0.bm, l0.bn, l0.stages);
+    if (!grouped) {
+        for (int i = 0; i < n; ++i) {
+            const int e = prx_gemm_launch(d[i], ws, ws_bytes, stream, ctx);
+            if (e) return e;
+        }
+        return 0;
+    }
+    GemmGroupArg<1> grp{};
+    for (int i = 0; i < n; ++i) { grp.A[i] = d[i].A; grp.B[i] = d[i].B; grp.out_f32[i] = d[i].out_f32; grp.out_bf16[i] = d[i].out_bf16; }
+    const int e = launch_planned(d[0], l0, ws, n_cu, stream, ctx, &grp, n);
+    if (e) return e;
+    g_group_launches.fetch_add(1, std::memory_order_relaxed);
+    return 0;
+}
diff --git a/pixray_amd/csrc/gemm_epi.h b/pixray_amd/csrc/gemm_epi.h
--- a/pixray_amd/csrc/gemm_epi.h
+++ b/pixray_amd/csrc/gemm_epi.h
@@ -12,6 +12,17 @@
     int fit_flags;
     float* ws;
 };
+
+constexpr int GEMM_GROUP_MAX = 4;
+template <int GROUP>
+struct GemmGroupArg {
+    const void* A[GEMM_GROUP_MAX];
+    const void* B[GEMM_GROUP_MAX];
+    float* out_f32[GEMM_GROUP_MAX];
+    void* out_bf16[GEMM_GROUP_MAX];
+};
+template <>
+struct GemmGroupArg<0> {};
 
 __device__ __forceinline__ float quickgelu_f(float t) { return t * sigmoidf_(1.702f * t); }
 __device__ __forceinline__ float dquickgelu_f(float t) {
diff --git a/pixray_amd/csrc/vqgan.hip b/pixray_amd/csrc/vqgan.hip
--- a/pixray_amd/csrc/vqgan.hip
+++ b/pixray_amd/csrc/vqgan.hip
@@ -85,6 +85,7 @@
     int prec;
     int f32, h16;
     int lean;
+    int attn_group;
     float* gs;
     GemmCtx gctx;
     DevArena mem;
@@ -218,6 +219,7 @@
     v->prec = precision; v->f32 = prec_is_f32(precision); v->h16 = prec_is_h16(precision);
     v->gs = nullptr;
     { const char* e = getenv("PRX_LEAN"); v->lean = (v->h16 && !(e && atoi(e) == 0)) ? 1 : 0; }
+    { const char* e = getenv("PRX_VQ_ATTN_GROUP"); v->attn_group = (e && atoi(e) == 0) ? 0 : 1; }
     v->n_gn = 0; v->zc = z_channels; v->D = embed_dim; v->NC = n_embed; v->ch = ch; v->out_ch = out_ch; v->h0 = h0; v->w0 = w0;
     WCursor cur{w, n_w, 0};
     int r;
@@ -333,12 +335,15 @@
     fprintf(stderr, "[vq] %s %2d n=%zu l2 %.9e max %.6e\n", tag, i, n, sqrt(q), mx);
 }
 
-static int vg(PrxVqgan* v, GemmDesc& d, hipStream_t s) {
+static void vg_prec(const PrxVqgan* v, GemmDesc& d) {
     if (v->f32) {
         d.f32 = 1; d.a_is_f32 = 0;
         if (d.out_bf16 == (void*)d.out_f32) d.out_bf16 = nullptr;
     }
     d.h16 = v->h16;
+}
+static int vg(PrxVqgan* v, GemmDesc& d, hipStream_t s) {
+    vg_prec(v, d);
     return prx_gemm_launch(d, v->ws, v->ws_bytes, s, &v->gctx);
 }
 GemmCtx* prx_vqgan_gemm_ctx_impl(PrxVqgan* v) { return v ? &v->gctx : nullptr; }
@@ -451,11 +456,12 @@
                 d.bias_n = b.qkv.b; d.out_bf16 = b.qkvb; d.ldc_bf16 = 3 * C;
                 if ((r = vg(v, d, s))) return r; }
             const int P8 = pad8(P);
-            if ((r = prx_transpose_op(b.qkvb, 3 * C, b.qkvT, P8, P, 3 * C, v->f32, s))) return r;
+            if (!v->attn_group && (r = prx_transpose_op(b.qkvb, 3 * C, b.qkvT, P8, P, 3 * C, v->f32, s))) return r;
             {   GemmDesc d; d.A = b.qkvb; d.lda = 3 * C; d.B = op_off(b.qkvb, C, v->f32); d.ldb = 3 * C; d.M = P; d.N = P; d.K = C;
                 d.out_f32 = v->S; d.ldc_f32 = P;
                 if ((r = vg(v, d, s))) return r; }
-            if ((r = prx_softmax_rows(v->S, P, 1.f / sqrtf((float)C), b.Pm, P8, b.PT, P8, P, P, v->prec, s))) return r;
+            if (v->attn_group) { if ((r = prx_softmax_rows_tr(v->S, P, 1.f / sqrtf((float)C), b.Pm, P8, b.PT, P8, P, P, b.qkvb, 3 * C, b.qkvT, P8, P, 3 * C, v->prec, s))) return r; }
+            else if ((r = prx_softmax_rows(v->S, P, 1.f / sqrtf((float)C), b.Pm, P8, b.PT, P8, P, P, v->prec, s))) return r;
             {   GemmDesc d; d.A = b.Pm; d.lda = P8; d.B = op_off(b.qkvT, (size_t)2 * C * P8, v->f32); d.ldb = P8; d.M = P; d.N = C; d.K = P8;
                 d.out_bf16 = v->tB; d.ldc_bf16 = C;
                 if ((r = vg(v, d, s))) return r; }
@@ -553,18 +559,27 @@
             const int P8 = pad8(P);
             if ((r = zero_if_padded(v, v->tB, P, P, s))) return r;
             if ((r = zero_if_padded(v, v->tC, P, P, s))) return r;
-            if ((r = prx_softmax_rows_bwd(b.Pm, P8, v->S, P, 1.f / sqrtf((float)C), v->tB, P8, v->tC, P8, P, P, v->prec, s))) return r;
-            {   GemmDesc d; d.A = v->tB; d.lda = P8; d.B = op_off(b.qkvT, (size_t)C * P8, v->f32); d.ldb = P8; d.M = P; d.N = C; d.K = P8;
-                d.out_bf16 = v->dqkv; d.ldc_bf16 = 3 * C;
-                if ((r = vg(v, d, s))) return r; }
-            {   GemmDesc d; d.A = v->tC; d.lda = P8; d.B = b.qkvT; d.ldb = P8; d.M = P; d.N = C; d.K = P8;
-                d.out_bf16 = op_off(v->dqkv, C, v->f32); d.ldc_bf16 = 3 * C;
-                if ((r = vg(v, d, s))) return r; }
-            if ((r = zero_if_padded(v, v->tD, C, P, s))) return r;
-            if ((r = prx_transpose_op(v->tA, C, v->tD, P8, P, C, v->f32, s))) return r;
-            {   GemmDesc d; d.A = b.PT; d.lda = P8; d.B = v->tD; d.ldb = P8; d.M = P; d.N = C; d.K = P8;
-                d.out_bf16 = op_off(v->dqkv, 2 * C, v->f32); d.ldc_bf16 = 3 * C;
-                if ((r = vg(v, d, s))) return r; }
+            GemmDesc dq, dk, dv;
+            dq.A = v->tB; dq.lda = P8; dq.B = op_off(b.qkvT, (size_t)C * P8, v->f32); dq.ldb = P8; dq.M = P; dq.N = C; dq.K = P8;
+            dq.out_bf16 = v->dqkv; dq.ldc_bf16 = 3 * C;
+            dk.A = v->tC; dk.lda = P8; dk.B = b.qkvT; dk.ldb = P8; dk.M = P; dk.N = C; dk.K = P8;
+            dk.out_bf16 = op_off(v->dqkv, C, v->f32); dk.ldc_bf16 = 3 * C;
+            dv.A = b.PT; dv.lda = P8; dv.B = v->tD; dv.ldb = P8; dv.M = P; dv.N = C; dv.K = P8;
+            dv.out_bf16 = op_off(v->dqkv, 2 * C, v->f32); dv.ldc_bf16 = 3 * C;
+            if (v->attn_group) {
+                if ((r = zero_if_padded(v, v->tD, C, P, s))) return r;
+                if ((r = prx_softmax_rows_bwd_tr(b.Pm, P8, v->S, P, 1.f / sqrtf((float)C), v->tB, P8, v->tC, P8, P, P, v->tA, C, v->tD, P8, P, C, v->prec, s))) return r;
+                GemmDesc grp[3] = {dq, dk, dv};
+                for (GemmDesc& d : grp) vg_prec(v, d);
+                if ((r = prx_gemm_launch_group(grp, 3, v->ws, v->ws_bytes, s, &v->gctx))) return r;
+            } else {
+                if ((r = prx_softmax_rows_bwd(b.Pm, P8, v->S, P, 1.f / sqrtf((float)C), v->tB, P8, v->tC, P8, P, P, v->prec, s))) return r;
+                if ((r = vg(v, dq, s))) return r;
+                if ((r = vg(v, dk, s))) return r;
+                if ((r = zero_if_padded(v, v->tD, C, P, s))) return r;
+                if ((r = prx_transpose_op(v->tA, C, v->tD, P8, P, C, v->f32, s))) return r;
+                if ((r = vg(v, dv, s))) return r;
+            }
             {   GemmDesc d; d.A = v->dqkv; d.lda = 3 * C; d.B = b.qkv.WT; d.ldb = 3 * C; d.M = P; d.N = C; d.K = 3 * C;
                 out_stream(v, d, t1.f, C, nullptr);
                 set_gnb(v, d, &b.n, b.x_in, 0);
```

Measured after the change: 171.7 (median of 6 runs). 1.3% higher.
